# sulaimanvesal/PointCloudUDA

Measured on AMD Instinct MI355X. Metric: adversarial train-step images/sec (seg+3 discr) at 256x256, higher is better.
Workload: dtype bf16x3 MFMA (split-bf16, fp32 accumulate; fp32 storage); 1 GPU; MS-CMRSeg full UDA: UNet(PointNet head) + d1 + d2 + d4, 256x256x1, 4 classes; per_gpu_batch=32, global_batch=32, precision=bf16x3, parallelism=dp1, ranks_in_group=1, collective=none, streams=discriminators concurrent, d_target_forward=replayed from the adversarial pass of the same step, launch=eager (256 host cores for this rank)

## Files before the change

include/pcuda_hip.h:

```cpp
#ifndef PCUDA_HIP_H
#define PCUDA_HIP_H

#include <stddef.h>
#include <stdint.h>

#ifdef __cplusplus
extern "C" {
#endif

#define PCUDA_OK 0
#define PCUDA_E_BADARG (-1)
#define PCUDA_E_UNSUPPORTED (-2)
#define PCUDA_E_LAUNCH (-3)
#define PCUDA_E_WORKSPACE (-4)

#define PCUDA_PREC_BF16X3 0
#define PCUDA_PREC_BF16 1

typedef void* pcuda_stream_t;

#define PCUDA_ABI_VERSION 5
int pcuda_version(void);
size_t pcuda_abi_struct_size(int which);
int pcuda_device_count(void);
const char* pcuda_last_error(void);
const char* pcuda_build_hash(void);
long long pcuda_launch_count(int reset);
long long pcuda_fallback_count(void);
const char* pcuda_last_kernel(void);
int pcuda_clock_probe(unsigned long long* out2_dev, float* sink_dev, int iters, pcuda_stream_t s);

#define PCUDA_FAM_CONV_FWD 0
#define PCUDA_FAM_CONV_WGRAD 1
#define PCUDA_FAM_POINTWISE 2
#define PCUDA_FAM_DENSE_F32 3
#define PCUDA_FAM_COUNT 4
int pcuda_prof_enable(int on);
int pcuda_prof_reset(void);
int pcuda_prof_read(int family, double* ms, double* work, long long* launches);
int pcuda_prof_dump(const char* path);
int pcuda_debug_read_clocks(unsigned long long* out8);

typedef struct pcuda_conv_geom {
  int n;
  int cin, cout;
  int in_h, in_w;
  int out_h, out_w;
  int k, stride, pad, dil;
  int in_up;
} pcuda_conv_geom;

typedef struct pcuda_src {
  const float* p1; long long sn1, sc1; const float* scale1; const float* shift1;
  const float* p2; long long sn2, sc2; const float* scale2; const float* shift2;
  int c1;
} pcuda_src;
typedef struct pcuda_dst {
  float* p1; long long sn1, sc1;
  float* p2; long long sn2, sc2;
  int c1;
} pcuda_dst;

size_t pcuda_conv2d_packed_fwd_bytes(const pcuda_conv_geom* g, int prec);
size_t pcuda_conv2d_packed_dgrad_bytes(const pcuda_conv_geom* g, int prec);
int pcuda_conv2d_pack_fwd(const pcuda_conv_geom* g, int prec, const float* w, void* packed, pcuda_stream_t s);
int pcuda_conv2d_pack_dgrad(const pcuda_conv_geom* g, int prec, const float* w, void* packed, pcuda_stream_t s);
int pcuda_conv2d_pack_all(const pcuda_conv_geom* g, int prec, const float* w, void* packed_fwd, void* packed_dgrad,
                          pcuda_stream_t s);
size_t pcuda_conv2d_pack_job_bytes(void);
int pcuda_conv2d_pack_jobs_fill(const pcuda_conv_geom* g, int prec, const float* w, void* packed_fwd, void* packed_dgrad,
                                void* host_jobs, int max_jobs, int* job_blocks);
int pcuda_conv2d_pack_table(const void* dev_jobs, const int* dev_first_block, int njobs, int total_blocks, pcuda_stream_t s);

int pcuda_conv2d_d1_forward_ok(const pcuda_conv_geom* g);
int pcuda_conv2d_fwd_tiles(const pcuda_conv_geom* g, int prec);
int pcuda_conv2d_forward(const pcuda_conv_geom* g, int prec, const pcuda_src* x, const void* packed_w,
                         const float* bias, float slope, const pcuda_dst* y, float* bn_partials,
                         pcuda_stream_t s);
int pcuda_conv2d_dgrad(const pcuda_conv_geom* g, int prec, const pcuda_src* dy, const void* packed_w_dgrad,
                       const pcuda_dst* dx, int accumulate, pcuda_stream_t s);
int pcuda_conv2d_dgrad_tiles(const pcuda_conv_geom* g, int prec);
int pcuda_conv2d_dgrad_bnred(const pcuda_conv_geom* g, int prec, const pcuda_src* dy, const void* packed_w_dgrad,
                             const pcuda_dst* dx, int accumulate, const float* a, long long a_sn, long long a_sc,
                             const float* mean, const float* invstd, float* red_partials, pcuda_stream_t s);
int pcuda_conv2d_dgrad_lrelu(const pcuda_conv_geom* g, int prec, const pcuda_src* dy, const void* packed_w_dgrad,
                             const pcuda_dst* dx, const float* a, long long a_sn, long long a_sc, float slope,
                             pcuda_stream_t s);
int pcuda_conv2d_dgrad_fold(const pcuda_conv_geom* g, int prec, const pcuda_src* dy, const void* packed_w_dgrad,
                            const pcuda_dst* dx_half, const float* a, long long a_sn, long long a_sc, const float* mean,
                            const float* invstd, float* red_partials, pcuda_stream_t s);
size_t pcuda_conv2d_wgrad_workspace_size(const pcuda_conv_geom* g);
int pcuda_conv2d_wgrad(const pcuda_conv_geom* g, int prec, const pcuda_src* x, const float* dy,
                       long long dy_sn, long long dy_sc, float* dw, float* db, int accumulate,
                       void* workspace, size_t workspace_bytes, pcuda_stream_t s);

#define PCUDA_REDUCE_MAX_JOBS 56
typedef struct {
  const float* partial;
  long long numel;
  float* dw;
  const float* db_partial;
  long long nb;
  float* db;
  int ksplit, nkg, accumulate, ntaps;
} pcuda_reduce_job;
int pcuda_conv2d_wgrad_partial(const pcuda_conv_geom* g, int prec, const pcuda_src* x, const float* dy,
                               long long dy_sn, long long dy_sc, float* dw, float* db, int accumulate,
                               void* workspace, size_t workspace_bytes, pcuda_reduce_job* job, pcuda_stream_t s);
int pcuda_wgrad_reduce_batch(const pcuda_reduce_job* host_jobs, int njobs, pcuda_stream_t s);

int pcuda_bn_finalize(const float* partials, int ntiles, int c, long long count, const float* gamma,
                      const float* beta, float eps, float momentum, float* running_mean, float* running_var,
                      float* mean, float* invstd, float* scale, float* shift, pcuda_stream_t s);
int pcuda_bn_stats(const float* a, long long sn, long long sc, int n, int c, long long hw,
                   float* partials, int* ntiles, pcuda_stream_t s);
#define PCUDA_BN_APPLY_RELU 1
#define PCUDA_BN_APPLY_FMA 2
int pcuda_bn_apply(const float* a, long long a_sn, long long a_sc, const float* scale, const float* shift,
                   int flags, float* y, long long y_sn, long long y_sc, int n, int c, long long hw,
                   pcuda_stream_t s);
int pcuda_bn_bwd_reduce(const float* dy, long long dy_sn, long long dy_sc, const float* dy2, long long dy2_sn,
                        long long dy2_sc, const float* a, long long a_sn, long long a_sc, const float* mean,
                        const float* invstd, const float* scale, const float* shift, int post_relu, int n, int c,
                        long long hw, float* red, int* ntiles, pcuda_stream_t s);
int pcuda_bn_bwd_finalize(const float* red, int ntiles, int c, long long count, const float* gamma,
                          const float* invstd, const float* mean, float* dgamma, float* dbeta, int accumulate,
                          float* coef , pcuda_stream_t s);
int pcuda_bn_bwd_apply(const float* dy, long long dy_sn, long long dy_sc, const float* dy2, long long dy2_sn,
                       long long dy2_sc, const float* a, long long a_sn, long long a_sc, const float* coef,
                       const float* scale, const float* shift, int post_relu, float act_slope, float* dz,
                       long long dz_sn, long long dz_sc, int n, int c, long long hw, pcuda_stream_t s);
int pcuda_lrelu_bwd(const float* dy, long long dy_sn, long long dy_sc, const float* dy2, long long dy2_sn,
                    long long dy2_sc, const float* a, long long a_sn, long long a_sc, float slope, float* dz,
                    long long dz_sn, long long dz_sc, int n, int c, long long hw, pcuda_stream_t s);
int pcuda_channel_sum(const float* dz, long long sn, long long sc, int n, int c, long long hw, float* db,
                      int accumulate, float* workspace, size_t workspace_bytes, pcuda_stream_t s);

int pcuda_maxpool2_fwd(const float* x, long long x_sn, long long x_sc, const float* scale, const float* shift,
                       float* y, long long y_sn, long long y_sc, uint8_t* idx, int n, int c, int h, int w,
                       pcuda_stream_t s);
int pcuda_maxpool2_bwd(const float* dy, long long dy_sn, long long dy_sc, const float* dy2, long long dy2_sn,
                       long long dy2_sc, const uint8_t* idx, float* dx, long long dx_sn, long long dx_sc,
                       int accumulate, int n, int c, int h, int w, pcuda_stream_t s);
typedef struct pcuda_pooled {
  const float* g; long long g_sn, g_sc;
  const float* g2; long long g2_sn, g2_sc;
  const uint8_t* idx;
  int h, w;
} pcuda_pooled;
int pcuda_bn_bwd_reduce_pooled(const pcuda_pooled* pool, const float* dy, long long dy_sn, long long dy_sc, const float* a,
                               long long a_sn, long long a_sc, const float* mean, const float* invstd, int n, int c,
                               float* red, int* ntiles, pcuda_stream_t s);
int pcuda_bn_bwd_apply_pooled(const pcuda_pooled* pool, const float* dy, long long dy_sn, long long dy_sc, const float* a,
                              long long a_sn, long long a_sc, const float* coef, float act_slope, float* dz, long long dz_sn,
                              long long dz_sc, int n, int c, pcuda_stream_t s);
int pcuda_lrelu_bwd_pooled(const pcuda_pooled* pool, const float* dy, long long dy_sn, long long dy_sc, const float* a,
                           long long a_sn, long long a_sc, float slope, float* dz, long long dz_sn, long long dz_sc, int n,
                           int c, pcuda_stream_t s);
int pcuda_upsample2_bwd(const float* dy, long long dy_sn, long long dy_sc, float* dx, long long dx_sn,
                        long long dx_sc, int accumulate, int n, int c, int h, int w, pcuda_stream_t s);
int pcuda_upsample2_bwd_bnred(const float* dy, long long dy_sn, long long dy_sc, float* dx, long long dx_sn,
                              long long dx_sc, int accumulate, const float* a, long long a_sn, long long a_sc,
                              const float* mean, const float* invstd, float* red, int* ntiles, int n, int c, int h, int w,
                              pcuda_stream_t s);
int pcuda_bilinear_fwd(const float* x, long long x_sn, long long x_sc, int n, int c, int h, int w, float* y, int oh,
                       int ow, pcuda_stream_t s);
int pcuda_bilinear_bwd(const float* dy, int n, int c, int oh, int ow, float* dx, long long dx_sn, long long dx_sc,
                       int h, int w, pcuda_stream_t s);
int pcuda_unfold_taps(const float* x, long long x_sn, long long x_sc, int n, int c, int h, int w, int k, int stride,
                      int pad, int dil, float* u, int oh, int ow, pcuda_stream_t s);
int pcuda_add4(const float* a, const float* b, const float* c, const float* d, float* y, long long numel,
               pcuda_stream_t s);
int pcuda_mul(const float* a, const float* b, float* y, long long numel, pcuda_stream_t s);

#define PCUDA_ACT_SIGMOID 0
#define PCUDA_ACT_SOFTMAX 1
int pcuda_entropy_fwd(const float* logits, int mode, float norm, float* ent, float* prob, int n, int c,
                      long long hw, pcuda_stream_t s);
int pcuda_entropy_bwd(const float* logits, int mode, float norm, const float* dent, const float* dprob,
                      float* dlogits, int accumulate, int n, int c, long long hw, pcuda_stream_t s);
int pcuda_entropy_bwd2(const float* logits, int mode, float norm, const float* dent, const float* dprob, const float* dmean,
                       float* dlogits, int accumulate, int n, int c, long long hw, pcuda_stream_t s);
size_t pcuda_sum_all_workspace_size(void);
int pcuda_sum_all(const float* x, long long numel, double scale, float* out, void* workspace, size_t workspace_bytes,
                  pcuda_stream_t s);
size_t pcuda_seg_loss_workspace_size(int n, int c, long long hw);
int pcuda_seg_loss_fwd(const float* logits, const uint8_t* onehot, int mode, int n, int c, long long hw,
                       float* out2, void* workspace, size_t workspace_bytes, pcuda_stream_t s);
int pcuda_seg_loss_bwd(const float* logits, const uint8_t* onehot, int mode, int n, int c, long long hw,
                       const float* g_main, const float* g_jac, float* dlogits, const void* workspace,
                       pcuda_stream_t s);
int pcuda_bce_const_fwd(const float* x, long long numel, float label, float* loss, float* acc, pcuda_stream_t s);
int pcuda_bce_const_bwd(const float* x, long long numel, float label, const float* gout, float gscale, float* dx,
                        pcuda_stream_t s);
size_t pcuda_nn_loss_workspace_floats(int b, int npts);
int pcuda_nn_loss_fwd(const float* x, const float* y, int b, int npts, float* loss, int* idx_ws, float* val_ws,
                      pcuda_stream_t s);
int pcuda_nn_loss_bwd(const float* x, const float* y, int b, int npts, const int* idx_ws, const float* val_ws,
                      const float* gout, float* dx, pcuda_stream_t s);
int pcuda_dice_metric(const float* logits, const uint8_t* onehot, int n, int c, long long hw, float* dice,
                      void* workspace, size_t workspace_bytes, pcuda_stream_t s);
int pcuda_assemble_batch(const float* images_hwc, const int* mask_labels, int b, int h, int w, int c, int crop,
                         int num_classes, float* images_chw, uint8_t* onehot, pcuda_stream_t s);
size_t pcuda_minmax_workspace_size(void);
int pcuda_minmax(const float* x, long long numel, float* out2, void* workspace, size_t workspace_bytes, pcuda_stream_t s);
int pcuda_quantize_u8(const float* x, long long numel, const float* minmax, uint8_t* q, pcuda_stream_t s);
#define PCUDA_AUG_NONE 0
#define PCUDA_AUG_MINMAX 1
#define PCUDA_AUG_DIV255 2
int pcuda_augment_assemble(const void* images_hwc, int images_u8, const int* mask_labels, int b, int h, int w, int c, int crop,
                           int num_classes, const double* inv_mats, const int* order, const int* cval, int rescale,
                           const float* minmax, float* images_chw, uint8_t* onehot, uint8_t* full_mask, int* labels_full,
                           uint8_t* images_u8_full, pcuda_stream_t s);
int pcuda_augment_assemble_dequant(const uint8_t* images_hwc, const int* mask_labels, int b, int h, int w, int c, int crop,
                                   int num_classes, const double* inv_mats, const int* order, const int* cval,
                                   const float* minmax, float* images_chw, uint8_t* onehot, uint8_t* full_mask,
                                   int* labels_full, uint8_t* images_u8_full, pcuda_stream_t s);
#define PCUDA_PHOTO_NOP 0
#define PCUDA_PHOTO_GAUSSIAN_BLUR 1
#define PCUDA_PHOTO_AVERAGE_BLUR 2
#define PCUDA_PHOTO_MEDIAN_BLUR 3
#define PCUDA_PHOTO_CONV3X3 4
#define PCUDA_PHOTO_GAUSSIAN_NOISE 5
#define PCUDA_PHOTO_DROPOUT 6
#define PCUDA_PHOTO_COARSE_DROPOUT 7
#define PCUDA_PHOTO_INVERT 8
#define PCUDA_PHOTO_ADD 9
#define PCUDA_PHOTO_MULTIPLY 10
#define PCUDA_PHOTO_GRAYSCALE 11
size_t pcuda_photometric_workspace_size(int b, int h, int w, int c);
int pcuda_photometric(const uint8_t* in, uint8_t* out, int b, int h, int w, int c, int slots, const int* opcode,
                      const int* iarg, const double* farg, const unsigned long long* seed, void* workspace,
                      size_t workspace_bytes, pcuda_stream_t s);
#define PCUDA_GEO_NOP 0
#define PCUDA_GEO_HOMOGRAPHY 1
#define PCUDA_GEO_ELASTIC 2
#define PCUDA_GEO_PIECEWISE_AFFINE 3
#define PCUDA_GEO_CONSTANT 0
#define PCUDA_GEO_EDGE 1
#define PCUDA_GEO_REFLECT 2
#define PCUDA_GEO_SYMMETRIC 3
#define PCUDA_GEO_WRAP 4
size_t pcuda_geometric_workspace_size(int b, int h, int w, int c, int with_labels);
int pcuda_geometric(const uint8_t* in, uint8_t* out, const int* labels_in, int* labels_out, int b, int h, int w, int c,
                    int slots, const int* opcode, const int* iarg, const double* farg, const unsigned long long* seed,
                    void* workspace, size_t workspace_bytes, pcuda_stream_t s);
int pcuda_geometric_cubic(const uint8_t* in, uint8_t* out, const int* labels_in, int* labels_out, int b, int h, int w, int c,
                          int slots, const int* opcode, const int* iarg, const double* farg, const unsigned long long* seed,
                          void* workspace, size_t workspace_bytes, pcuda_stream_t s);
#define PCUDA_STYLE_NOP 0
#define PCUDA_STYLE_HUE_SATURATION 1
#define PCUDA_STYLE_NOISE_ALPHA_CONV3X3 2
#define PCUDA_STYLE_SUPERPIXELS 3
size_t pcuda_stylize_workspace_size(int b, int h, int w, int c);
int pcuda_stylize(const uint8_t* in, uint8_t* out, int b, int h, int w, int c, int slots, const int* opcode, const int* iarg,
                  const double* farg, const double* table, const unsigned long long* seed, void* workspace,
                  size_t workspace_bytes, pcuda_stream_t s);
size_t pcuda_stylize_connect_workspace_size(int b, int h, int w, int c);
int pcuda_stylize_connect(const uint8_t* in, uint8_t* out, int b, int h, int w, int c, int slots, const int* opcode,
                          const int* iarg, const double* farg, const double* table, const unsigned long long* seed,
                          void* workspace, size_t workspace_bytes, pcuda_stream_t s);
size_t pcuda_stylize_scaled_workspace_size(int b, int h, int w, int c);
int pcuda_stylize_scaled(const uint8_t* in, uint8_t* out, int b, int h, int w, int c, int slots, const int* opcode,
                         const int* iarg, const double* farg, const double* table, const unsigned long long* seed,
                         void* workspace, size_t workspace_bytes, pcuda_stream_t s);
#define PCUDA_PAD_CONSTANT 0
#define PCUDA_PAD_EDGE 1
#define PCUDA_PAD_LINEAR_RAMP 2
#define PCUDA_PAD_MAXIMUM 3
#define PCUDA_PAD_MEAN 4
#define PCUDA_PAD_MEDIAN 5
#define PCUDA_PAD_MINIMUM 6
#define PCUDA_PAD_REFLECT 7
#define PCUDA_PAD_SYMMETRIC 8
#define PCUDA_PAD_WRAP 9
size_t pcuda_crop_pad_workspace_size(int b, int h, int w, int c);
int pcuda_crop_pad(const uint8_t* in, uint8_t* out, const int* labels_in, int* labels_out, int b, int h, int w, int c,
                   const int* opcode, const int* iarg, void* workspace, size_t workspace_bytes, pcuda_stream_t s);
size_t pcuda_match_hist_workspace_size(int b, int h, int w, int c, int is_u8);
int pcuda_match_hist(const void* in, void* out, int is_u8, int b, int h, int w, int c, const double* tvalues,
                     const double* tquantiles, const int* tlen, int tstride, void* workspace, size_t workspace_bytes,
                     pcuda_stream_t s);
size_t pcuda_hist_bank_size(int r, int rh, int rw, int c, int is_u8);
size_t pcuda_hist_bank_workspace_size(int r, int rh, int rw, int c, int is_u8);
int pcuda_hist_bank_build(const void* refs, int is_u8, int r, int rh, int rw, int c, void* bank, size_t bank_bytes, int* flag,
                          void* workspace, size_t workspace_bytes, pcuda_stream_t s);
size_t pcuda_match_hist_bank_workspace_size(int b, int h, int w, int c, int is_u8);
int pcuda_match_hist_bank(const void* in, void* out, int is_u8, int b, int h, int w, int c, const void* bank, int r, int rh,
                          int rw, const int* ref_index, void* workspace, size_t workspace_bytes, pcuda_stream_t s);
size_t pcuda_fourier_bank_size(int r, int c, int radius);
size_t pcuda_fourier_bank_workspace_size(int r, int h, int w, int c, int radius);
int pcuda_fourier_bank_build(const void* refs, int is_u8, int r, int h, int w, int c, int radius, void* bank, size_t bank_bytes,
                             void* workspace, size_t workspace_bytes, pcuda_stream_t s);
size_t pcuda_fourier_adapt_workspace_size(int b, int h, int w, int c, int radius);
int pcuda_fourier_adapt(const void* in, void* out, int is_u8, int b, int h, int w, int c, const void* bank, int r, int radius,
                        const int* ref_index, const int* sample_radius, int clip, double clip_lo, double clip_hi, void* workspace,
                        size_t workspace_bytes, pcuda_stream_t s);
#define PCUDA_CLAHE_U8 0
#define PCUDA_CLAHE_F32X3 1
#define PCUDA_PRE_F32 0
#define PCUDA_PRE_I16 1
#define PCUDA_PRE_U8 2
#define PCUDA_PRE_U8_RAW 3
size_t pcuda_clahe_workspace_size(int n, int tiles_x, int tiles_y);
int pcuda_clahe(const uint8_t* in, void* out, int n, int h, int w, double clip_limit, int tiles_x, int tiles_y, int out_mode,
                void* workspace, size_t workspace_bytes, pcuda_stream_t s);
size_t pcuda_rescale_resize_crop_u8_workspace_size(void);
int pcuda_rescale_resize_crop_u8(const void* in, int in_dtype, int n, int sh, int sw, int resize_h, int resize_w, int crop,
                                 uint8_t* out, void* workspace, size_t workspace_bytes, pcuda_stream_t s);
size_t pcuda_zoom_linear_crop_workspace_size(int zh, int zw, int crop);
int pcuda_zoom_linear_crop(const void* in, int dtype, int n, int sh, int sw, int zh, int zw, int crop, void* out,
// ... 132 lines not shown
```

pointcloududa_amd/_lib.py:

```python
from __future__ import annotations

import ctypes as C
import os

_HERE = os.path.dirname(os.path.abspath(__file__))
LIB_PATH = os.environ.get("PCUDA_LIB") or os.path.join(_HERE, "lib", "libpcuda_hip.so")

PREC_BF16X3, PREC_BF16 = 0, 1
ACT_SIGMOID, ACT_SOFTMAX = 0, 1
OV_DICE_CLASS, OV_DICE_SAMPLE = 1, 2
FAM_CONV_FWD, FAM_CONV_WGRAD, FAM_POINTWISE, FAM_DENSE_F32 = 0, 1, 2, 3

c_f32p = C.c_void_p
i32, i64, f32, f64, vp, sz = C.c_int, C.c_longlong, C.c_float, C.c_double, C.c_void_p, C.c_size_t


class ConvGeom(C.Structure):
    _fields_ = [("n", i32), ("cin", i32), ("cout", i32), ("in_h", i32), ("in_w", i32), ("out_h", i32),
                ("out_w", i32), ("k", i32), ("stride", i32), ("pad", i32), ("dil", i32), ("in_up", i32)]


class ReduceJob(C.Structure):
    _fields_ = [("partial", C.c_void_p), ("numel", C.c_longlong), ("dw", C.c_void_p), ("db_partial", C.c_void_p),
                ("nb", C.c_longlong), ("db", C.c_void_p), ("ksplit", C.c_int), ("nkg", C.c_int), ("accumulate", C.c_int),
                ("ntaps", C.c_int)]


class Src(C.Structure):
    _fields_ = [("p1", vp), ("sn1", i64), ("sc1", i64), ("scale1", vp), ("shift1", vp),
                ("p2", vp), ("sn2", i64), ("sc2", i64), ("scale2", vp), ("shift2", vp), ("c1", i32)]


class Dst(C.Structure):
    _fields_ = [("p1", vp), ("sn1", i64), ("sc1", i64), ("p2", vp), ("sn2", i64), ("sc2", i64), ("c1", i32)]


class Pooled(C.Structure):
    _fields_ = [("g", vp), ("g_sn", i64), ("g_sc", i64), ("g2", vp), ("g2_sn", i64), ("g2_sc", i64), ("idx", vp),
                ("h", i32), ("w", i32)]


_PROTOS = {
    "pcuda_version": (i32, []),
    "pcuda_device_count": (i32, []),
    "pcuda_last_error": (C.c_char_p, []),
    "pcuda_build_hash": (C.c_char_p, []),
    "pcuda_launch_count": (i64, [i32]),
    "pcuda_fallback_count": (i64, []),
    "pcuda_abi_struct_size": (sz, [i32]),
    "pcuda_last_kernel": (C.c_char_p, []),
    "pcuda_clock_probe": (i32, [vp, vp, i32, vp]),
    "pcuda_prof_enable": (i32, [i32]),
    "pcuda_prof_reset": (i32, []),
    "pcuda_prof_read": (i32, [i32, C.POINTER(C.c_double), C.POINTER(C.c_double), C.POINTER(i64)]),
    "pcuda_prof_dump": (i32, [C.c_char_p]),
    "pcuda_debug_read_clocks": (i32, [vp]),
    "pcuda_conv2d_packed_fwd_bytes": (sz, [C.POINTER(ConvGeom), i32]),
    "pcuda_conv2d_packed_dgrad_bytes": (sz, [C.POINTER(ConvGeom), i32]),
    "pcuda_conv2d_pack_fwd": (i32, [C.POINTER(ConvGeom), i32, vp, vp, vp]),
    "pcuda_conv2d_pack_all": (i32, [C.POINTER(ConvGeom), i32, vp, vp, vp, vp]),
    "pcuda_conv2d_pack_dgrad": (i32, [C.POINTER(ConvGeom), i32, vp, vp, vp]),
    "pcuda_conv2d_pack_job_bytes": (sz, []),
    "pcuda_conv2d_pack_jobs_fill": (i32, [C.POINTER(ConvGeom), i32, vp, vp, vp, vp, i32, C.POINTER(i32)]),
    "pcuda_conv2d_pack_table": (i32, [vp, vp, i32, i32, vp]),
    "pcuda_conv2d_fwd_tiles": (i32, [C.POINTER(ConvGeom), i32]),
    "pcuda_conv2d_forward": (i32, [C.POINTER(ConvGeom), i32, C.POINTER(Src), vp, vp, f32, C.POINTER(Dst), vp, vp]),
    "pcuda_conv2d_d1_forward_ok": (i32, [C.POINTER(ConvGeom)]),
    "pcuda_conv2d_dgrad": (i32, [C.POINTER(ConvGeom), i32, C.POINTER(Src), vp, C.POINTER(Dst), i32, vp]),
    "pcuda_conv2d_dgrad_tiles": (i32, [C.POINTER(ConvGeom), i32]),
    "pcuda_conv2d_dgrad_bnred": (i32, [C.POINTER(ConvGeom), i32, C.POINTER(Src), vp, C.POINTER(Dst), i32, vp, i64, i64, vp,
                                       vp, vp, vp]),
    "pcuda_conv2d_dgrad_fold": (i32, [C.POINTER(ConvGeom), i32, C.POINTER(Src), vp, C.POINTER(Dst), vp, i64, i64, vp, vp, vp, vp]),
    "pcuda_conv2d_dgrad_lrelu": (i32, [C.POINTER(ConvGeom), i32, C.POINTER(Src), vp, C.POINTER(Dst), vp, i64, i64, f32, vp]),
    "pcuda_conv2d_wgrad_workspace_size": (sz, [C.POINTER(ConvGeom)]),
    "pcuda_conv2d_wgrad": (i32, [C.POINTER(ConvGeom), i32, C.POINTER(Src), vp, i64, i64, vp, vp, i32, vp, sz, vp]),
    "pcuda_conv2d_wgrad_partial": (i32, [C.POINTER(ConvGeom), i32, C.POINTER(Src), vp, i64, i64, vp, vp, i32, vp, sz,
                                         C.POINTER(ReduceJob), vp]),
    "pcuda_wgrad_reduce_batch": (i32, [C.POINTER(ReduceJob), i32, vp]),
    "pcuda_bn_finalize": (i32, [vp, i32, i32, i64, vp, vp, f32, f32, vp, vp, vp, vp, vp, vp, vp]),
    "pcuda_bn_stats": (i32, [vp, i64, i64, i32, i32, i64, vp, C.POINTER(i32), vp]),
    "pcuda_bn_apply": (i32, [vp, i64, i64, vp, vp, i32, vp, i64, i64, i32, i32, i64, vp]),
    "pcuda_bn_bwd_reduce": (i32, [vp, i64, i64, vp, i64, i64, vp, i64, i64, vp, vp, vp, vp, i32, i32, i32, i64, vp,
                                  C.POINTER(i32), vp]),
    "pcuda_bn_bwd_finalize": (i32, [vp, i32, i32, i64, vp, vp, vp, vp, vp, i32, vp, vp]),
    "pcuda_bn_bwd_apply": (i32, [vp, i64, i64, vp, i64, i64, vp, i64, i64, vp, vp, vp, i32, f32, vp, i64, i64, i32,
                                 i32, i64, vp]),
    "pcuda_lrelu_bwd": (i32, [vp, i64, i64, vp, i64, i64, vp, i64, i64, f32, vp, i64, i64, i32, i32, i64, vp]),
    "pcuda_channel_sum": (i32, [vp, i64, i64, i32, i32, i64, vp, i32, vp, sz, vp]),
    "pcuda_maxpool2_fwd": (i32, [vp, i64, i64, vp, vp, vp, i64, i64, vp, i32, i32, i32, i32, vp]),
    "pcuda_maxpool2_bwd": (i32, [vp, i64, i64, vp, i64, i64, vp, vp, i64, i64, i32, i32, i32, i32, i32, vp]),
    "pcuda_bn_bwd_reduce_pooled": (i32, [C.POINTER(Pooled), vp, i64, i64, vp, i64, i64, vp, vp, i32, i32, vp, C.POINTER(i32), vp]),
    "pcuda_bn_bwd_apply_pooled": (i32, [C.POINTER(Pooled), vp, i64, i64, vp, i64, i64, vp, f32, vp, i64, i64, i32, i32, vp]),
    "pcuda_lrelu_bwd_pooled": (i32, [C.POINTER(Pooled), vp, i64, i64, vp, i64, i64, f32, vp, i64, i64, i32, i32, vp]),
    "pcuda_upsample2_bwd": (i32, [vp, i64, i64, vp, i64, i64, i32, i32, i32, i32, i32, vp]),
    "pcuda_upsample2_bwd_bnred": (i32, [vp, i64, i64, vp, i64, i64, i32, vp, i64, i64, vp, vp, vp, C.POINTER(i32), i32, i32,
                                        i32, i32, vp]),
    "pcuda_bilinear_fwd": (i32, [vp, i64, i64, i32, i32, i32, i32, vp, i32, i32, vp]),
    "pcuda_bilinear_bwd": (i32, [vp, i32, i32, i32, i32, vp, i64, i64, i32, i32, vp]),
    "pcuda_unfold_taps": (i32, [vp, i64, i64, i32, i32, i32, i32, i32, i32, i32, i32, vp, i32, i32, vp]),
    "pcuda_add4": (i32, [vp, vp, vp, vp, vp, i64, vp]),
    "pcuda_mul": (i32, [vp, vp, vp, i64, vp]),
    "pcuda_entropy_fwd": (i32, [vp, i32, f32, vp, vp, i32, i32, i64, vp]),
    "pcuda_entropy_bwd": (i32, [vp, i32, f32, vp, vp, vp, i32, i32, i32, i64, vp]),
    "pcuda_entropy_bwd2": (i32, [vp, i32, f32, vp, vp, vp, vp, i32, i32, i32, i64, vp]),
    "pcuda_sum_all_workspace_size": (sz, []),
    "pcuda_sum_all": (i32, [vp, i64, C.c_double, vp, vp, sz, vp]),
    "pcuda_seg_loss_workspace_size": (sz, [i32, i32, i64]),
    "pcuda_seg_loss_fwd": (i32, [vp, vp, i32, i32, i32, i64, vp, vp, sz, vp]),
    "pcuda_seg_loss_bwd": (i32, [vp, vp, i32, i32, i32, i64, vp, vp, vp, vp, vp]),
    "pcuda_jaccard_workspace_size": (sz, [i32]),
    "pcuda_jaccard_fwd": (i32, [vp, vp, i32, i32, i32, i64, f32, vp, vp, sz, vp]),
    "pcuda_jaccard_bwd": (i32, [vp, i32, i32, i32, i64, f32, vp, vp, vp, vp]),
    "pcuda_seg_loss_ov_workspace_size": (sz, [i32, i32, i64, i32]),
    "pcuda_seg_loss_ov_fwd": (i32, [vp, vp, i32, i32, C.c_double, i32, i32, i64, vp, vp, sz, vp]),
    "pcuda_seg_loss_ov_bwd": (i32, [vp, vp, i32, i32, i32, i32, i64, vp, vp, vp, vp, sz, vp]),
    "pcuda_dice_workspace_size": (sz, [i32, i32, i64, i32]),
    "pcuda_dice_fwd": (i32, [vp, vp, i32, i32, i32, i64, i32, f32, vp, vp, sz, vp]),
    "pcuda_dice_bwd": (i32, [vp, i32, i32, i32, i64, i32, vp, vp, vp, sz, vp]),
    "pcuda_dice_labels_workspace_size": (sz, [i32, i32, i64]),
    "pcuda_dice_labels_fwd": (i32, [vp, vp, i32, i32, i32, i64, f32, vp, vp, vp, sz, vp]),
    "pcuda_dice_labels_bwd": (i32, [vp, vp, i32, i32, i32, i64, vp, vp, vp, sz, vp]),
    "pcuda_bce_const_fwd": (i32, [vp, i64, f32, vp, vp, vp]),
    "pcuda_bce_const_bwd": (i32, [vp, i64, f32, vp, f32, vp, vp]),
    "pcuda_nn_loss_workspace_floats": (sz, [i32, i32]),
    "pcuda_nn_loss_fwd": (i32, [vp, vp, i32, i32, vp, vp, vp, vp]),
    "pcuda_nn_loss_bwd": (i32, [vp, vp, i32, i32, vp, vp, vp, vp, vp]),
    "pcuda_dice_metric": (i32, [vp, vp, i32, i32, i64, vp, vp, sz, vp]),
    "pcuda_assemble_batch": (i32, [vp, vp, i32, i32, i32, i32, i32, i32, vp, vp, vp]),
    "pcuda_minmax_workspace_size": (sz, []),
    "pcuda_minmax": (i32, [vp, i64, vp, vp, sz, vp]),
    "pcuda_augment_assemble": (i32, [vp, i32, vp, i32, i32, i32, i32, i32, i32, vp, vp, vp, i32, vp, vp, vp, vp, vp, vp, vp]),
    "pcuda_quantize_u8": (i32, [vp, i64, vp, vp, vp]),
    "pcuda_augment_assemble_dequant": (i32, [vp, vp, i32, i32, i32, i32, i32, i32, vp, vp, vp, vp, vp, vp, vp, vp, vp, vp]),
    "pcuda_photometric_workspace_size": (sz, [i32, i32, i32, i32]),
    "pcuda_photometric": (i32, [vp, vp, i32, i32, i32, i32, i32, vp, vp, vp, vp, vp, sz, vp]),
    "pcuda_geometric_workspace_size": (sz, [i32, i32, i32, i32, i32]),
    "pcuda_geometric": (i32, [vp, vp, vp, vp, i32, i32, i32, i32, i32, vp, vp, vp, vp, vp, sz, vp]),
    "pcuda_geometric_cubic": (i32, [vp, vp, vp, vp, i32, i32, i32, i32, i32, vp, vp, vp, vp, vp, sz, vp]),
    "pcuda_stylize_workspace_size": (sz, [i32, i32, i32, i32]),
    "pcuda_stylize": (i32, [vp, vp, i32, i32, i32, i32, i32, vp, vp, vp, vp, vp, vp, sz, vp]),
    "pcuda_stylize_connect_workspace_size": (sz, [i32, i32, i32, i32]),
    "pcuda_stylize_connect": (i32, [vp, vp, i32, i32, i32, i32, i32, vp, vp, vp, vp, vp, vp, sz, vp]),
    "pcuda_stylize_scaled_workspace_size": (sz, [i32, i32, i32, i32]),
    "pcuda_stylize_scaled": (i32, [vp, vp, i32, i32, i32, i32, i32, vp, vp, vp, vp, vp, vp, sz, vp]),
    "pcuda_crop_pad_workspace_size": (sz, [i32, i32, i32, i32]),
    "pcuda_crop_pad": (i32, [vp, vp, vp, vp, i32, i32, i32, i32, vp, vp, vp, sz, vp]),
    "pcuda_match_hist_workspace_size": (sz, [i32, i32, i32, i32, i32]),
    "pcuda_match_hist": (i32, [vp, vp, i32, i32, i32, i32, i32, vp, vp, vp, i32, vp, sz, vp]),
    "pcuda_hist_bank_size": (sz, [i32, i32, i32, i32, i32]),
    "pcuda_hist_bank_workspace_size": (sz, [i32, i32, i32, i32, i32]),
    "pcuda_hist_bank_build": (i32, [vp, i32, i32, i32, i32, i32, vp, sz, vp, vp, sz, vp]),
    "pcuda_match_hist_bank_workspace_size": (sz, [i32, i32, i32, i32, i32]),
    "pcuda_match_hist_bank": (i32, [vp, vp, i32, i32, i32, i32, i32, vp, i32, i32, i32, vp, vp, sz, vp]),
    "pcuda_fourier_bank_size": (sz, [i32, i32, i32]),
    "pcuda_fourier_bank_workspace_size": (sz, [i32, i32, i32, i32, i32]),
    "pcuda_fourier_bank_build": (i32, [vp, i32, i32, i32, i32, i32, i32, vp, sz, vp, sz, vp]),
    "pcuda_fourier_adapt_workspace_size": (sz, [i32, i32, i32, i32, i32]),
    "pcuda_fourier_adapt": (i32, [vp, vp, i32, i32, i32, i32, i32, vp, i32, i32, vp, vp, i32, f64, f64, vp, sz, vp]),
    "pcuda_clahe_workspace_size": (sz, [i32, i32, i32]),
    "pcuda_clahe": (i32, [vp, vp, i32, i32, i32, f64, i32, i32, i32, vp, sz, vp]),
    "pcuda_rescale_resize_crop_u8_workspace_size": (sz, []),
    "pcuda_rescale_resize_crop_u8": (i32, [vp, i32, i32, i32, i32, i32, i32, i32, vp, vp, sz, vp]),
    "pcuda_zoom_linear_crop_workspace_size": (sz, [i32, i32, i32]),
    "pcuda_zoom_linear_crop": (i32, [vp, i32, i32, i32, i32, i32, i32, i32, vp, vp, sz, vp]),
    "pcuda_zoom_standardize_workspace_size": (sz, [i32, i32, i32, i32, i32]),
    "pcuda_zoom_standardize": (i32, [vp, i32, i32, i32, i32, i32, i32, i32, i32, vp, vp, vp, sz, vp]),
    "pcuda_zoom_labels_workspace_size": (sz, [i32, i32, i32]),
    "pcuda_zoom_labels": (i32, [vp, i32, i32, i32, i32, i32, i32, i32, i32, vp, i32, vp, vp, sz, vp]),
    "pcuda_volume_slices": (i32, [vp, i32, i64, i64, i64, i64, i32, i32, i32, i32, i32, i32, vp, vp]),
    "pcuda_volume_labels_workspace_size": (sz, []),
    "pcuda_volume_labels": (i32, [vp, i32, i64, i64, i64, i64, i32, i32, i32, i32, i32, i32, vp, i32, i32, vp, vp, vp, sz, vp]),
    "pcuda_volume_restore": (i32, [vp, i32, i32, i32, vp, i32, i64, i64, i64, i64, i32, i32, vp, vp]),
    "pcuda_argmax_labels": (i32, [vp, i32, i64, i64, i32, i32, i64, vp, vp]),
    "pcuda_label_dice": (i32, [vp, vp, i64, i32, vp, vp, sz, vp]),
    "pcuda_area_resize": (i32, [vp, i64, i64, i32, i32, i32, vp, i32, i32, vp]),
    "pcuda_reconstruct_resize_argmax": (i32, [vp, i64, i64, i64, i32, i32, i32, i32, i32, i32, vp, i32, i32, vp]),
    "pcuda_surface_metrics_workspace_size": (sz, [i32, i32, i32, i32, i32, vp]),
    "pcuda_surface_metrics": (i32, [vp, vp, i32, i32, i32, i32, i32, vp, i32, i32, vp, vp, vp, sz, vp]),
    "pcuda_surface_metrics_ext_workspace_size": (sz, [i32, i32, i32, i32, i32, vp]),
    "pcuda_surface_metrics_ext": (i32, [vp, vp, i32, i32, i32, i32, i32, vp, i32, i32, vp, f64, vp, vp, sz, vp]),
    "pcuda_largest_components_workspace_size": (sz, [i32, i32, i32, i32]),
    "pcuda_largest_components": (i32, [vp, i32, i32, i32, i32, i32, i32, vp, vp, sz, vp]),
    "pcuda_linear_fwd": (i32, [vp, vp, vp, vp, i32, i32, i32, vp]),
    "pcuda_linear_bwd_x": (i32, [vp, vp, vp, i32, i32, i32, i32, vp]),
    "pcuda_linear_bwd_w_workspace_size": (sz, [i32, i32, i32]),
    "pcuda_linear_bwd_w": (i32, [vp, vp, vp, vp, i32, i32, i32, i32, vp, sz, vp]),
    "pcuda_conv1d_k1_fwd_tiles": (i32, [i32, i32]),
    "pcuda_conv1d_k1_fwd": (i32, [vp, vp, vp, vp, i32, i32, i32, i32, vp, vp]),
    "pcuda_conv1d_k1_dgrad": (i32, [vp, vp, vp, i32, i32, i32, i32, vp]),
    "pcuda_conv1d_k1_wgrad_workspace_size": (sz, [i32, i32, i32, i32]),
    "pcuda_conv1d_k1_wgrad": (i32, [vp, vp, vp, vp, i32, i32, i32, i32, i32, vp, sz, vp]),
    "pcuda_max_points_fwd": (i32, [vp, i32, i32, i32, vp, vp, vp]),
    "pcuda_max_points_bwd": (i32, [vp, vp, i32, i32, i32, vp, vp]),
    "pcuda_bn1d_fwd": (i32, [vp, i64, i32, i32, vp, vp, f32, f32, vp, vp, vp, vp, vp, vp, i32, vp, i64, vp]),
    "pcuda_bn1d_bwd": (i32, [vp, i64, vp, i64, i32, i32, vp, vp, vp, vp, vp, i32, f32, vp, vp, i32, vp, i64, vp]),
    "pcuda_bn_bwd_reduce_maxpts": (i32, [vp, vp, vp, vp, vp, vp, vp, i32, i32, i32, i32, vp, vp]),
    "pcuda_bn_bwd_apply_maxpts": (i32, [vp, vp, vp, vp, vp, vp, i32, f32, vp, i32, i32, i32, vp]),
    "pcuda_bmm": (i32, [vp, vp, vp, i32, i32, i32, i32, i32, i32, i32, vp]),
    "pcuda_surface_vertices": (i32, [vp, i32, i32, i32, vp, i32, vp, vp, sz, vp]),
    "pcuda_surface_vertices_mc": (i32, [vp, i32, i32, i32, vp, i32, vp, vp]),
    "pcuda_fps": (i32, [vp, vp, vp, i32, i32, i32, vp, vp]),
    "pcuda_adam_step": (i32, [vp, vp, vp, vp, i64, f32, f32, f32, f32, f32, i32, f32, vp]),
    "pcuda_adam_step_dev": (i32, [vp, vp, vp, vp, i64, f32, f32, f32, f32, f32, vp, f32, vp]),
    "pcuda_sgd_step": (i32, [vp, vp, vp, i64, f32, f32, f32, i32, f32, vp]),
    "pcuda_grad_norm": (i32, [vp, C.POINTER(i64), i32, f32, f32, i32, vp, vp, vp, sz, vp]),
    "pcuda_adam_step_guarded": (i32, [vp, vp, vp, vp, i64, f32, f32, f32, f32, f32, vp, f32, vp, i32, vp]),
    "pcuda_sgd_step_guarded": (i32, [vp, vp, vp, i64, f32, f32, f32, vp, i32, f32, vp, i32, vp]),
}

EXPORTED_SYMBOLS = tuple(_PROTOS.keys())
_lib = None


PCUDA_E_UNSUPPORTED = -2
PCUDA_ABI_VERSION = 5
GUARD_MAX_RANGES, GUARD_RECORD_WORDS, GRAD_NORM_WORKSPACE_BYTES = 16, 8, 16384


def lib():
    global _lib
    if _lib is None:
        if not os.path.exists(LIB_PATH):
            raise RuntimeError("libpcuda_hip.so is missing at %s: build it with pointcloududa_amd/csrc/Makefile "
                               "(there is no CPU fallback)" % LIB_PATH)
        handle = C.CDLL(LIB_PATH)
        for name, (res, args) in _PROTOS.items():
            fn = getattr(handle, name)
            fn.restype, fn.argtypes = res, args
        ver = handle.pcuda_version()
        if ver != PCUDA_ABI_VERSION:
            raise RuntimeError("libpcuda_hip.so at %s has ABI version %d, this binding is written against %d: rebuild it "
                               "(python -c 'import __graft_entry__ as g; g.build()')" % (LIB_PATH, ver, PCUDA_ABI_VERSION))
        for which, st in enumerate((ConvGeom, Src, Dst, Pooled, ReduceJob)):
            if handle.pcuda_abi_struct_size(which) != C.sizeof(st):
                raise RuntimeError("libpcuda_hip.so: sizeof(%s) is %d in the library, %d in the binding: header / library mismatch"
                                   % (st.__name__, handle.pcuda_abi_struct_size(which), C.sizeof(st)))
        _lib = handle
    return _lib


def source_hash(csrc: str) -> str:
    import glob
    import hashlib
    h = hashlib.sha256()
    files = sorted(glob.glob(os.path.join(csrc, "*.hip")) + glob.glob(os.path.join(csrc, "*.h")) +
                   [os.path.join(csrc, "Makefile"), os.path.join(os.path.dirname(os.path.dirname(csrc)), "include", "pcuda_hip.h")])
# ... 24 lines not shown
```

pointcloududa_amd/csrc/conv_host.h:

```cpp
#pragma once
#include <stdlib.h>
#include <string.h>
#include "conv_igemm.h"

static const int LDS_HARD = 160 * 1024;

static inline bool geom_ok(const pcuda_conv_geom* g) {
  if (!g || g->n <= 0 || g->cin <= 0 || g->cout <= 0 || g->k <= 0 || g->stride <= 0 || g->dil <= 0 || g->pad < 0)
    return false;
  if (g->k * g->k > IG_MAX_TAPS) return false;
  const int oh = (g->in_h + 2 * g->pad - g->dil * (g->k - 1) - 1) / g->stride + 1;
  const int ow = (g->in_w + 2 * g->pad - g->dil * (g->k - 1) - 1) / g->stride + 1;
  if (oh != g->out_h || ow != g->out_w || oh <= 0 || ow <= 0) return false;
  if (g->in_up && ((g->in_h & 1) || (g->in_w & 1))) return false;
  return true;
}

static inline bool src_ok(const pcuda_src* s, int c) {
  if (!s || !s->p1 || s->c1 <= 0 || s->c1 > c) return false;
  if (s->c1 < c && !s->p2) return false;
  return true;
}
static inline bool dst_ok(const pcuda_dst* d, int c) {
  if (!d || !d->p1 || d->c1 <= 0 || d->c1 > c) return false;
  if (d->c1 < c && !d->p2) return false;
  return true;
}

struct TapSet {
  int n;
  signed char dy[IG_MAX_TAPS], dx[IG_MAX_TAPS], src[IG_MAX_TAPS];
  int dy_min, dy_max, dx_min, dx_max;
  void finish() {
    dy_min = dx_min = 127; dy_max = dx_max = -127;
    for (int i = 0; i < n; ++i) {
      if (dy[i] < dy_min) dy_min = dy[i];
      if (dy[i] > dy_max) dy_max = dy[i];
      if (dx[i] < dx_min) dx_min = dx[i];
      if (dx[i] > dx_max) dx_max = dx[i];
    }
    if (n == 0) dy_min = dy_max = dx_min = dx_max = 0;
  }
};

static inline TapSet fwd_taps(const pcuda_conv_geom* g) {
  TapSet t = {};
  for (int ky = 0; ky < g->k; ++ky)
    for (int kx = 0; kx < g->k; ++kx) {
      t.dy[t.n] = (signed char)(ky * g->dil - g->pad);
      t.dx[t.n] = (signed char)(kx * g->dil - g->pad);
      t.src[t.n] = (signed char)(ky * g->k + kx);
      ++t.n;
    }
  t.finish();
  return t;
}

static inline int posmod(int a, int m) { return ((a % m) + m) % m; }

static inline TapSet dgrad_taps(const pcuda_conv_geom* g, int ry, int rx) {
  TapSet t = {};
  const int s = g->stride;
  for (int ky = 0; ky < g->k; ++ky) {
    const int vy = ry + g->pad - ky * g->dil;
    if (posmod(vy, s) != 0) continue;
    for (int kx = 0; kx < g->k; ++kx) {
      const int vx = rx + g->pad - kx * g->dil;
      if (posmod(vx, s) != 0) continue;
      t.dy[t.n] = (signed char)(vy / s);
      t.dx[t.n] = (signed char)(vx / s);
      t.src[t.n] = (signed char)(ky * g->k + kx);
      ++t.n;
    }
  }
  t.finish();
  return t;
}

static inline bool dgrad_pair_enabled() {
  static int on = -1;
  if (on < 0) { const char* e = getenv("PCUDA_DGRAD_PAIR"); on = (e && !atoi(e)) ? 0 : 1; }
  return on != 0;
}
static inline bool dgrad_pair_ok(const pcuda_conv_geom* g) {
  if (g->stride != 2 || g->in_up || g->cin <= 5 || !dgrad_pair_enabled()) return false;
  for (int ry = 0; ry < 2; ++ry) {
    const TapSet a = dgrad_taps(g, ry, 0), b = dgrad_taps(g, ry, 1);
    if (a.n < 1 || a.n != b.n || 2 * a.n > IG_MAX_TAPS) return false;
    for (int i = 0; i < a.n; ++i)
      if (a.dy[i] != b.dy[i] || a.dx[i] != b.dx[i]) return false;
  }
  return true;
}
static inline TapSet dgrad_pair_taps(const pcuda_conv_geom* g, int ry) {
  TapSet t = dgrad_taps(g, ry, 0);
  const TapSet b = dgrad_taps(g, ry, 1);
  for (int i = 0; i < b.n; ++i) t.src[t.n + i] = b.src[i];
  return t;
}

static inline int tile_width_candidates(int lw, int tile_px, int* out) {
  int n = 0;
  for (int t = 8; t <= 256 && t <= tile_px; t <<= 1) out[n++] = t;
  for (int parts = 1; parts <= 4; ++parts) {
    const int t = (lw + parts - 1) / parts;
    if (t >= 4 && t <= 256 && t <= tile_px) {
      bool dup = false;
      for (int i = 0; i < n; ++i) dup |= out[i] == t;
      if (!dup) out[n++] = t;
    }
  }
  return n;
}


static inline bool fast_src_ok(const pcuda_src* x, int cin) {
  const long long lim = 1ll << 30;
  const int c1 = x->c1 < cin ? x->c1 : cin;
  if (c1 < cin && (c1 & 31)) return false;
  if ((long long)(c1 + 32) * x->sc1 * 4 >= lim) return false;
  if (c1 < cin && (long long)(cin - c1 + 32) * x->sc2 * 4 >= lim) return false;
  return true;
}

static inline bool aligned16(const void* p, long long sn, long long sc) { return (((uintptr_t)p) & 15) == 0 && (sn & 3) == 0 && (sc & 3) == 0; }

static inline bool fast_dst_ok(const pcuda_dst* y, int cout) {
  const long long lim = 1ll << 30;
  const int c1 = y->c1 < cout ? y->c1 : cout;
  if (c1 < cout && (c1 & 7)) return false;
  if ((long long)(c1 + 64) * y->sc1 * 4 >= lim) return false;
  if (c1 < cout && (long long)(cout - c1 + 64) * y->sc2 * 4 >= lim) return false;
  return true;
}

struct IgemmPlan {
  int npb, tw, th, tiles_x, tiles_y, ih_t, iw_t, clamp, x_cap, tg;
  size_t lds;
  int fat;
  int w8;
  int te;
};

static inline bool te_dst_ok(const pcuda_dst* y, int cout, int out_w, int lw, int tw, int ox_mul, int ox_off) {
  if (ox_mul != 1 || ox_off != 0 || (tw & 3) || (out_w & 3) || (lw & 3)) return false;
  if (((uintptr_t)y->p1 & 15) || (y->sc1 & 3) || (y->sn1 & 3)) return false;
  if (y->c1 < cout && (((uintptr_t)y->p2 & 15) || (y->sc2 & 3) || (y->sn2 & 3))) return false;
  return true;
}


struct IgemmParams;
struct PackParams;
bool ap_layer_ok(const pcuda_conv_geom* g, int rows, int red, int prec);
size_t ap_layer_packed_bytes(int rows, int red);
bool ap_fill_pack(PackParams& p, const float* w, unsigned char* out, int rows, int red, long long s_row, long long s_red,
                  const TapSet& taps);
int ap_launch_pack(const float* w, unsigned char* out, int rows, int red, long long s_row, long long s_red, const TapSet& taps,
                   hipStream_t s);
bool ap_map_ok(int n, int h, int w, int rows);
int ap_tiles(int n, int h, int w);
int ap_try_launch(const IgemmParams& p, const TapSet& taps, const unsigned char* image, hipStream_t s, int* rc);

bool rs_layer_ok(const pcuda_conv_geom* g, int rows, int red, int prec);
bool rs_map_ok(int n, int h, int w);
int rs_tiles(int n, int h, int w);
int rs_try_launch(const IgemmParams& p, int prec, const TapSet& taps, hipStream_t s, int* rc);

static inline size_t packed_elems(int rows, int red, int ntaps, int prec) {
  const int co_tile = 32 * ig_co_blks(rows);
  const int n_co_tiles = cdiv(rows, co_tile), nchunks = cdiv(red, 32);
  return (size_t)n_co_tiles * nchunks * ntaps * co_tile * (ig_rec_bytes(prec == PCUDA_PREC_BF16X3) / 2);
}

enum { SIDE_FWD = 0, SIDE_DGRAD = 1 };
enum { IMG_ORDINARY = 0, IMG_PAIR = 1, IMG_AP = 2 };
struct PackedImage {
  int kind;
  int rows, red;
  long long s_row, s_red;
  int ry, rx;
  size_t off, bytes;
  TapSet taps;
};
struct PackedLayout {
  int n;
  size_t bytes;
  PackedImage img[IG_MAX_TAPS + 1];
  const PackedImage* ap() const { return n > 0 && img[n - 1].kind == IMG_AP ? &img[n - 1] : nullptr; }
  const PackedImage* cls(int ry, int rx) const {
    for (int i = 0; i < n; ++i)
      if (img[i].kind != IMG_AP && img[i].ry == ry && img[i].rx == rx) return &img[i];
    return nullptr;
  }
};
static inline void packed_layout(const pcuda_conv_geom* g, int prec, int side, PackedLayout* L) {
  const int kk = g->k * g->k;
  const bool fwd = side == SIDE_FWD;
  const int rows = fwd ? g->cout : g->cin, red = fwd ? g->cin : g->cout;
  const long long s_row = fwd ? (long long)g->cin * kk : kk, s_red = fwd ? kk : (long long)g->cin * kk;
  L->n = 0; L->bytes = 0;
  auto add = [&](int kind, int r, const TapSet& t, int ry, int rx) {
    PackedImage& im = L->img[L->n++];
    im.kind = kind; im.rows = r; im.red = red; im.s_row = s_row; im.s_red = s_red; im.ry = ry; im.rx = rx; im.taps = t;
    im.off = L->bytes;
    im.bytes = kind == IMG_AP ? ap_layer_packed_bytes(r, red) : packed_elems(r, red, t.n, prec) * 2;
    L->bytes += im.bytes;
  };
  if (fwd) {
    add(IMG_ORDINARY, rows, fwd_taps(g), 0, 0);
  } else if (dgrad_pair_ok(g)) {
    for (int ry = 0; ry < 2; ++ry) add(IMG_PAIR, 2 * rows, dgrad_pair_taps(g, ry), ry, 0);
    return;
  } else {
    for (int ry = 0; ry < g->stride; ++ry)
      for (int rx = 0; rx < g->stride; ++rx) {
        const TapSet t = dgrad_taps(g, ry, rx);
        if (t.n) add(IMG_ORDINARY, rows, t, ry, rx);
      }
  }
  if (ap_layer_ok(g, rows, red, prec)) add(IMG_AP, rows, L->img[0].taps, 0, 0);
}

int direct_fwd_tiles(const pcuda_conv_geom* g);
int direct_forward(const pcuda_conv_geom* g, int prec, const pcuda_src* x, const void* packed_w, long long w_lo_off,
                   const float* bias, float slope, const pcuda_dst* y, float* bn_partials, hipStream_t s, int* rc);
int direct_dgrad_tiles(const pcuda_conv_geom* g);
int direct_dgrad(const pcuda_conv_geom* g, int prec, const pcuda_src* dy, const void* packed_w_dgrad, const pcuda_dst* dx,
                 int accumulate, hipStream_t s, int* rc, const float* red_a = nullptr, long long red_sn = 0,
                 long long red_sc = 0, const float* red_mean = nullptr, const float* red_invstd = nullptr,
                 float* red = nullptr);
int direct_d1_dgrad(const pcuda_conv_geom* g, int prec, const pcuda_src* dy, const void* packed_w_dgrad, const pcuda_dst* dx,
                    int accumulate, size_t cls_elems, hipStream_t s, int* rc);
int direct_d1_forward(const pcuda_conv_geom* g, int prec, const pcuda_src* x, const void* packed_w, const float* bias,
                      float slope, const pcuda_dst* y, float* bn_partials, hipStream_t s, int* rc);
int direct_d5_forward(const pcuda_conv_geom* g, int prec, const pcuda_src* x, const void* packed_w, const float* bias,
                      float slope, const pcuda_dst* y, float* bn_partials, hipStream_t s, int* rc);

struct WgradCall {
  const pcuda_conv_geom* g;
  int prec;
  const pcuda_src* x;
  const float* dy;
  long long dy_sn, dy_sc;
  float* dw;
  float* db;
  int accumulate;
  void* workspace;
  hipStream_t s;
  pcuda_reduce_job* defer;
};
enum { WGRAD_NOT_TAKEN = 1 };

struct WgradSlabs {
  float* partial;
  float* db_partial;
  long long welems;
  int slices, ntaps;
};
static inline size_t wgrad_slab_bytes(const pcuda_conv_geom* g, int slices) {
  return ((size_t)slices * g->cout * g->cin * g->k * g->k + (size_t)slices * g->cout) * sizeof(float) + 256;
}
WgradSlabs wgrad_slabs(const WgradCall& c, int slices, int ntaps);
int wgrad_finish(const WgradCall& c, const WgradSlabs& sl);
int launch_wgrad_reduce(const float* partial, long long numel, int ksplit, float* dw, int accumulate, int ntaps,
                        const float* db_partial, long long nb, float* db, hipStream_t s);

int direct_wgrad_slices(const pcuda_conv_geom* g);
int direct_wgrad(const WgradCall& c);
size_t direct_d1_wgrad_bytes(const pcuda_conv_geom* g);
int direct_d1_wgrad(const WgradCall& c);
int wgrad3r_slices(const pcuda_conv_geom* g);
int wgrad3r_wgrad(const WgradCall& c);
int wgrad3_slices(const pcuda_conv_geom* g);
int wgrad3_wgrad(const WgradCall& c);
int wgrad1_slices(const pcuda_conv_geom* g);
int wgrad1_wgrad(const WgradCall& c);
```

pointcloududa_amd/csrc/conv_igemm.hip:

```cpp
#include <algorithm>
#include <stdlib.h>

#include "conv_igemm.h"
#include "conv_host.h"

#define PACK_MAX_JOBS 5
struct PackJobs {
  int n;
  PackParams p[PACK_MAX_JOBS];
};
__global__ void pack_multi_kernel(const PackJobs jobs) {
  const PackParams& p = jobs.p[blockIdx.y];
  const long long total = (long long)p.n_co_tiles * p.nchunks * p.ntaps * p.co_tile * p.rec;
  for (long long idx = blockIdx.x * (long long)blockDim.x + threadIdx.x; idx < total;
       idx += (long long)gridDim.x * blockDim.x) {
    int col = (int)(idx % p.rec);
    long long rest = idx / p.rec;
    int row = (int)(rest % p.co_tile); rest /= p.co_tile;
    int t = (int)(rest % p.ntaps); rest /= p.ntaps;
    int ch = (int)(rest % p.nchunks);
    int cot = (int)(rest / p.nchunks);
    const bool is_lo = p.rec > IG_REC && col >= 32;
    const int cc = is_lo ? col - 32 : col;
    int r = cot * p.co_tile + row, c = ch * 32 + cc;
// ... 135 lines not shown
  p.pair = im.kind == IMG_PAIR ? 1 : 0;
  memcpy(p.tap_src, im.taps.src, sizeof(p.tap_src));
  p.co_tile = 32 * ig_co_blks(im.rows);
  p.n_co_tiles = cdiv(im.rows, p.co_tile);
  p.nchunks = cdiv(im.red, 32);
  p.rec = ig_rec_bytes(prec == PCUDA_PREC_BF16X3) / 2;
  return true;
}

int launch_pack_jobs(const PackJobs& jobs, size_t max_elems, int max_blocks, hipStream_t s) {
  const int blocks = (int)std::min<size_t>((max_elems + 255) / 256, max_blocks);
  hipLaunchKernelGGL(pack_multi_kernel, dim3(blocks, jobs.n), dim3(256), 0, s, jobs);
  PCUDA_CHECK_LAUNCH("pack_multi_kernel");
  return PCUDA_OK;
}

int launch_pack(const float* w, void* buf, int prec, const PackedImage& im, hipStream_t s) {
  if (im.kind == IMG_AP)
    return ap_launch_pack(w, (unsigned char*)buf + im.off, im.rows, im.red, im.s_row, im.s_red, im.taps, s);
  PackJobs jobs = {};
  jobs.n = 1;
  fill_pack(jobs.p[0], w, buf, prec, im);
  return launch_pack_jobs(jobs, im.bytes / 2, 4096, s);
}

int pack_side(const pcuda_conv_geom* g, int prec, int side, const float* w, void* packed, hipStream_t s) {
  PackedLayout L;
  packed_layout(g, prec, side, &L);
  int rc = PCUDA_OK;
  for (int i = 0; i < L.n && rc == PCUDA_OK; ++i) rc = launch_pack(w, packed, prec, L.img[i], s);
  return rc;
}

int plan_lds(bool x3, int co_tile, int x_cap, int ntaps, int mode, int* tg_out, size_t* lds_out) {
  const bool fat = mode != 0;
  const size_t rec = ig_rec_bytes(x3), vecs = rec / 16;
  const size_t xb = (size_t)x_cap * rec;
  const size_t wtap = (size_t)co_tile * rec;
  const size_t epi = 4 * (size_t)co_tile * 2 * sizeof(float);
  const size_t tab = 1024;
  if (ntaps < 1) ntaps = 1;
  const int slots = mode == 2 ? (x3 ? 11 : 6) * 512 : (x3 ? (co_tile == 32 ? 8 : 7) : (co_tile == 32 ? 4 : 3)) * 256;
  const int cap = slots / (int)(co_tile * vecs);
  const size_t budgets[3] = {54528, 81920, 163840};
  for (int b = fat ? 2 : 0; b < 3; ++b) {
    if (xb + tab >= budgets[b]) continue;
    int fit = (int)((budgets[b] - xb - tab) / wtap);
    if (fit > cap) fit = cap;
    const int need = b == 0 ? (ntaps < 3 ? ntaps : 3) : 1;
    if (fit < need) continue;
    const int tg = fit > ntaps ? ntaps : fit;
    size_t total = xb + (size_t)tg * wtap + tab;
    if (total < epi) total = epi;
    *tg_out = tg; *lds_out = total;
    return 0;
  }
  return -1;
}


int plan_igemm_mode(int rows, int lh, int lw, int in_h, int in_w, int in_step, const TapSet& taps, bool x3,
                    int mode_env, IgemmPlan* best, int n = 0) {
  const int co_tile = 32 * ig_co_blks(rows);
  long long best_key = -1;
  for (int npb = 2; npb >= 1; --npb) {
    const int TP = 128 * npb;
    int cand[16];
    const int nc = tile_width_candidates(lw, TP, cand);
    for (int ci = 0; ci < nc; ++ci) {
      IgemmPlan pl;
      pl.npb = npb; pl.tw = cand[ci]; pl.th = TP / pl.tw;
      if (pl.th < 1) continue;
      pl.tiles_x = cdiv(lw, pl.tw);
      pl.tiles_y = cdiv(lh, pl.th);
      pl.ih_t = (pl.th - 1) * in_step + (taps.dy_max - taps.dy_min) + 1;
      pl.iw_t = (pl.tw - 1) * in_step + (taps.dx_max - taps.dx_min) + 1;
      const int full = pl.ih_t * pl.iw_t;
      const int clipped = (pl.ih_t < in_h ? pl.ih_t : in_h) * (pl.iw_t < in_w ? pl.iw_t : in_w) + 1;
      bool ok = false;
      for (int attempt = 0; attempt < 2 && !ok; ++attempt) {
        pl.clamp = attempt == 0 ? ((clipped * 2 <= full) ? 1 : 0) : 1;
        pl.x_cap = pl.clamp ? clipped : full;
        int mode = mode_env;
        if (mode == 2) {
          const int ihc = (pl.clamp && pl.ih_t > in_h) ? in_h : pl.ih_t;
          const bool fits = pl.x_cap <= 1024 && ihc * ((pl.iw_t + 6) / 4) <= 256;
          if (!fits || (npb == 1 && co_tile == 32)) mode = 0;
        }
        pl.fat = mode == 1 ? 1 : 0;
        pl.w8 = mode == 2 ? 1 : 0;
        ok = plan_lds(x3, co_tile, pl.x_cap, taps.n, mode, &pl.tg, &pl.lds) == 0;
        if (pl.clamp) break;
      }
      if (!ok) continue;
      const long long slots = (long long)pl.tiles_x * pl.tiles_y * TP;
      const long long halo = (long long)pl.x_cap * 64 / TP;
      const long long groups = (taps.n + pl.tg - 1) / pl.tg;
      const long long items = (long long)n * pl.tiles_x * pl.tiles_y * cdiv(rows, co_tile);
      static int nofill = -1;
      if (nofill < 0) { const char* e = getenv("PCUDA_NO_UNDERFILL"); nofill = (e && atoi(e)) ? 1 : 0; }
      const long long underfill = (!nofill && n > 0 && items < 256) ? (256 - items + 63) / 64 : 0;
      const long long key = (slots << 28) + (underfill << 25) + ((groups > 3 ? groups : 3) << 22) + ((pl.tw & 31) ? (1ll << 20) : 0) +
                            (halo << 8) + (npb == 1 ? 1 : 0);
      if (best_key < 0 || key < best_key) { best_key = key; *best = pl; }
    }
  }
  return best_key < 0 ? -1 : 0;
}

int plan_igemm(int rows, int red, int n, int lh, int lw, int in_h, int in_w, int in_step, const TapSet& taps, bool x3,
               IgemmPlan* best, bool allow8 = true) {
  const int mode_env = allow8 ? ig_plan_mode() : 0;
  const bool single_chunk = red <= 32;
  IgemmPlan p0;
  const int rc0 = plan_igemm_mode(rows, lh, lw, in_h, in_w, in_step, taps, x3, mode_env == 2 ? 0 : mode_env, &p0);
  if (mode_env != 2) { *best = p0; return rc0; }
  IgemmPlan p8;
  const int rc8 = plan_igemm_mode(rows, lh, lw, in_h, in_w, in_step, taps, x3, 2, &p8, n);
  if (rc8 < 0 || !p8.w8) { *best = p0; return rc0; }
  if (rc0 < 0) { *best = p8; return rc8; }
  const long long t0 = (long long)p0.tiles_x * p0.tiles_y, t8 = (long long)p8.tiles_x * p8.tiles_y;
  const long long items = (long long)n * (t0 < t8 ? t0 : t8) * cdiv(rows, 32 * ig_co_blks(rows));
  const bool wstay = rows <= 64 && taps.n <= p8.tg && single_chunk;
  const bool use8 = p0.lds > 81920 || items <= 320 || (wstay && ig_wstay_mode());
  *best = use8 ? p8 : p0;
  return 0;
}

enum { ROUTE_DIRECT, ROUTE_AP, ROUTE_RS, ROUTE_IGEMM };
struct ConvRoute {
  int family, tiles;
};
ConvRoute conv_route(const pcuda_conv_geom* g, int prec, int side, bool plan = true) {
  const bool fwd = side == SIDE_FWD;
  if (!fwd && g->stride != 1) return {ROUTE_IGEMM, 0};
  const int rows = fwd ? g->cout : g->cin, red = fwd ? g->cin : g->cout;
  if (const int d = fwd ? direct_fwd_tiles(g) : direct_dgrad_tiles(g)) return {ROUTE_DIRECT, d};
  if (ap_layer_ok(g, rows, red, prec) && ap_map_ok(g->n, g->in_h, g->in_w, rows)) return {ROUTE_AP, ap_tiles(g->n, g->in_h, g->in_w)};
  if (rs_layer_ok(g, rows, red, prec) && rs_map_ok(g->n, g->in_h, g->in_w)) return {ROUTE_RS, rs_tiles(g->n, g->in_h, g->in_w)};
  if (!plan) return {ROUTE_IGEMM, -1};
  IgemmPlan pl;
  const bool x3 = prec == PCUDA_PREC_BF16X3;
  const int rc = fwd ? plan_igemm(rows, red, g->n, g->out_h, g->out_w, g->in_h, g->in_w, g->stride, fwd_taps(g), x3, &pl)
                     : plan_igemm(rows, red, g->n, g->in_h, g->in_w, g->out_h, g->out_w, 1, dgrad_taps(g, 0, 0), x3, &pl);
  return {ROUTE_IGEMM, rc < 0 ? 0 : g->n * pl.tiles_x * pl.tiles_y};
}

int launch_igemm(IgemmParams& p, int prec, const TapSet& taps, hipStream_t s, const unsigned char* ap_image = nullptr,
                 const ConvRoute* expect = nullptr) {
  {
    int rc;
    if (ap_image && prec == PCUDA_PREC_BF16X3 && ap_try_launch(p, taps, ap_image, s, &rc)) return rc;
    if (p.cin == 32 && p.cout == 32 && rs_try_launch(p, prec, taps, s, &rc)) return rc;
  }
  const bool x3 = prec == PCUDA_PREC_BF16X3;
  const int co_blks = ig_co_blks(p.cout);
  const int co_tile = 32 * co_blks;
  IgemmPlan pl;
  if (plan_igemm(p.cout, p.cin, p.n, p.lh, p.lw, p.in_h, p.in_w, p.in_step, taps, x3, &pl, true) < 0)
    PCUDA_FAIL(PCUDA_E_UNSUPPORTED, "igemm: no tile of this convolution fits LDS (in_step %d, tap span %d)",
               p.in_step, taps.dy_max - taps.dy_min);
  if (p.stats && expect && expect->tiles >= 0 && (long long)pl.tiles_x * pl.tiles_y * p.n != expect->tiles)
    PCUDA_FAIL(PCUDA_E_UNSUPPORTED, "conv: tensors the %s kernel cannot address on a map whose ordinary plan has other tiles",
               expect->family == ROUTE_AP ? "anti-phase" : "row-streaming");
  p.n_co_tiles = cdiv(p.cout, co_tile);
  p.nchunks = cdiv(p.cin, 32);
  p.tw = pl.tw; p.th = pl.th; p.tmagic = 65536 / pl.tw + 1; p.tiles_x = pl.tiles_x; p.tiles_y = pl.tiles_y;
  auto fmagic = [](int d) -> unsigned { return d <= 1 ? 0u : (unsigned)((1ull << 32) / (unsigned)d) + 1u; };
  p.m_cot = fmagic(p.n_co_tiles); p.m_tx = fmagic(pl.tiles_x); p.m_ty = fmagic(pl.tiles_y);
  p.ntaps = taps.n;
  memcpy(p.dy, taps.dy, sizeof(p.dy));
  memcpy(p.dx, taps.dx, sizeof(p.dx));
  p.dy_min = taps.dy_min; p.dx_min = taps.dx_min;
  p.ih_t = pl.ih_t; p.iw_t = pl.iw_t; p.clamp = pl.clamp; p.tg = pl.tg;
  {
    static int dbg = -1;
    if (dbg < 0) { const char* e = getenv("PCUDA_DBG"); dbg = e ? atoi(e) : 0; }
    p.dbg = dbg;
    static unsigned long long* clkbuf = nullptr;
    if ((dbg & 128) && !clkbuf && hipMalloc((void**)&clkbuf, 64) == hipSuccess) (void)hipMemset(clkbuf, 0, 64);
    p.dbg_clk = clkbuf;
    g_dbg_clk_host = clkbuf;
  }
  const double flops = 2.0 * p.n * (double)p.lh * p.lw * p.cout * (double)p.cin * taps.n;
  char tag[160];
  snprintf(tag, sizeof(tag), "igemm n%d red%d rows%d %dx%d taps%d step%d up%d tw%d npb%d clamp%d tg%d w8%d lds%zu", p.n,
           p.cin, p.cout, p.lh, p.lw, taps.n, p.in_step, p.in_shift, pl.tw, pl.npb, pl.clamp, pl.tg, pl.w8, pl.lds);
  ProfScope prof(PCUDA_FAM_CONV_FWD, flops, s, tag);
  static int nopipe = -1;
  if (nopipe < 0) { const char* e = getenv("PCUDA_NOPIPE"); nopipe = e ? atoi(e) : 0; }
  const int max_pix = pl.clamp ? pl.x_cap - 1 : pl.ih_t * pl.iw_t;
  int pf = (max_pix + 255) / 256;
  {
    static int noxq = -1;
    if (noxq < 0) { const char* e = getenv("PCUDA_NOXQ"); noxq = e ? atoi(e) : 0; }
    const int ih = (pl.clamp && pl.ih_t > p.in_h) ? p.in_h : pl.ih_t;
    const int pfq = (ih * ((pl.iw_t + 6) / 4) + 63) / 64;
    p.xq = (!noxq && (p.in_w & 3) == 0 && p.in_shift == 0 && pfq <= 3) ? 1 : 0;
    if (p.xq) pf = pfq;
    if (pl.w8) pf = p.xq ? (ih * ((pl.iw_t + 6) / 4) + 127) / 128 : (max_pix + 511) / 512;
  }
  const long long total_items = (long long)p.n_co_tiles * p.n * pl.tiles_x * pl.tiles_y;
  const int max_div = std::max(p.n_co_tiles, std::max(pl.tiles_x, pl.tiles_y));
  const bool pipe = !nopipe && p.ntaps > 0 && fast_src_ok(&p.x, p.cin) && fast_dst_ok(&p.y, p.cout) &&
                    (pf <= 2 || (pf == 3 && !pl.w8 && (pl.npb == 1 || pl.fat))) && total_items < (1ll << 32) / max_div;
  {
    static int note = -1;
    if (note < 0) { const char* e = getenv("PCUDA_NOTE"); note = e ? atoi(e) : 0; }
    const bool fold_ok = p.fold && p.ox_mul == 1 && p.ox_off == 0 && !(pl.tw & 3) && !(p.lw & 3) && !(p.out_w & 1) &&
                         !((uintptr_t)p.y.p1 & 7) && !(p.y.sc1 & 1) && !(p.y.sn1 & 1) &&
                         (p.y.c1 >= p.cout || (!((uintptr_t)p.y.p2 & 7) && !(p.y.sc2 & 1) && !(p.y.sn2 & 1)));
    pl.te = (pipe && !pl.w8 && !note &&
             (p.fold ? fold_ok : te_dst_ok(&p.y, p.cout, p.out_w, p.lw, pl.tw, p.ox_mul, p.ox_off))) ? 1 : 0;
    if (pl.te) {
      const size_t rec = ig_rec_bytes(x3), wtap = (size_t)co_tile * rec;
      const size_t need = (size_t)16384 * pl.npb + (size_t)co_tile * 32;
      const size_t have = (size_t)pl.x_cap * rec + (size_t)pl.tg * wtap;
      if (have < need) {
        const int add = (int)((need - have + rec - 1) / rec);
        pl.x_cap += add;
        pl.lds += (size_t)add * rec;
      }
    }
  }
  if (p.fold && !(pipe && pl.te && !pl.w8 && pl.npb == 2 && pl.tw == 32 && pl.th == 8 && !pl.clamp && !p.accumulate && !p.pair))
    PCUDA_FAIL(PCUDA_E_UNSUPPORTED, "conv2d_dgrad_fold: this geometry does not run on the 32 x 8-tile transposed-epilogue kernel");
  if (p.mask_a && (pl.te || p.accumulate || p.stats || p.bias || p.fold || p.y.c1 < (p.cout >> p.pair)))
    PCUDA_FAIL(PCUDA_E_UNSUPPORTED, "conv2d_dgrad_lrelu: this geometry does not run on a plain-epilogue kernel");
  if (p.red_a && !(pipe && pl.te))
    PCUDA_FAIL(PCUDA_E_UNSUPPORTED, "conv2d_dgrad_bnred: this geometry does not run on the transposed-epilogue kernel");
  return x3 ? igemm_dispatch_x3(p, pl, co_blks, pf, pipe, s) : igemm_dispatch_bf16(p, pl, co_blks, pf, pipe, s);
}

}

static size_t packed_bytes(const pcuda_conv_geom* g, int prec, int side) {
  if (!geom_ok(g)) return 0;
  PackedLayout L;
  packed_layout(g, prec, side, &L);
  return L.bytes;
}
extern "C" size_t pcuda_conv2d_packed_fwd_bytes(const pcuda_conv_geom* g, int prec) { return packed_bytes(g, prec, SIDE_FWD); }
extern "C" size_t pcuda_conv2d_packed_dgrad_bytes(const pcuda_conv_geom* g, int prec) { return packed_bytes(g, prec, SIDE_DGRAD); }

extern "C" int pcuda_conv2d_pack_fwd(const pcuda_conv_geom* g, int prec, const float* w, void* packed,
                                     pcuda_stream_t s) {
  if (!geom_ok(g) || !w || !packed) PCUDA_FAIL(PCUDA_E_BADARG, "pack_fwd: bad geometry or null pointer");
  return pack_side(g, prec, SIDE_FWD, w, packed, (hipStream_t)s);
}

extern "C" int pcuda_conv2d_pack_dgrad(const pcuda_conv_geom* g, int prec, const float* w, void* packed,
                                       pcuda_stream_t s) {
  if (!geom_ok(g) || !w || !packed) PCUDA_FAIL(PCUDA_E_BADARG, "pack_dgrad: bad geometry or null pointer");
  return pack_side(g, prec, SIDE_DGRAD, w, packed, (hipStream_t)s);
}

extern "C" int pcuda_conv2d_pack_all(const pcuda_conv_geom* g, int prec, const float* w, void* packed_fwd,
                                     void* packed_dgrad, pcuda_stream_t s) {
  if (!geom_ok(g) || !w || !packed_fwd) PCUDA_FAIL(PCUDA_E_BADARG, "pack_all: bad geometry or null pointer");
  if (g->stride * g->stride + 1 > PACK_MAX_JOBS) {
    int rc = pcuda_conv2d_pack_fwd(g, prec, w, packed_fwd, s);
    if (rc == PCUDA_OK && packed_dgrad) rc = pcuda_conv2d_pack_dgrad(g, prec, w, packed_dgrad, s);
    return rc;
  }
  void* const buf[2] = {packed_fwd, packed_dgrad};
  PackedLayout L[2];
  PackJobs jobs = {};
  size_t max_elems = 0;
  for (int side = 0; side < 2 && buf[side]; ++side) {
    packed_layout(g, prec, side, &L[side]);
    for (int i = 0; i < L[side].n; ++i) {
      const PackedImage& im = L[side].img[i];
      if (im.kind == IMG_AP) continue;
      fill_pack(jobs.p[jobs.n++], w, buf[side], prec, im);
      max_elems = std::max(max_elems, im.bytes / 2);
    }
  }
  int rc = launch_pack_jobs(jobs, max_elems, 2048, (hipStream_t)s);
  for (int side = 0; side < 2 && buf[side] && rc == PCUDA_OK; ++side)
    if (const PackedImage* im = L[side].ap()) rc = launch_pack(w, buf[side], prec, *im, (hipStream_t)s);
  return rc;
}

extern "C" int pcuda_conv2d_fwd_tiles(const pcuda_conv_geom* g, int prec) {
  return geom_ok(g) ? conv_route(g, prec, SIDE_FWD).tiles : 0;
}

static IgemmParams dgrad_params(const pcuda_conv_geom* g, const pcuda_src* dy, const pcuda_dst* dx, const void* packed,
                                const PackedImage* im, int lh, int lw, int mul, int oy_off, int ox_off, int accumulate) {
  IgemmParams p;
  memset(&p, 0, sizeof(p));
  p.x = *dy; p.cin = g->cout;
  p.in_h = g->out_h; p.in_w = g->out_w; p.in_shift = 0; p.in_row = g->out_w;
  p.y = *dx; p.cout = im ? im->rows : g->cin; p.out_w = g->in_w;
  p.lh = lh; p.lw = lw;
  p.oy_mul = p.ox_mul = mul; p.oy_off = oy_off; p.ox_off = ox_off;
  p.in_step = 1;
  p.wpack = (const uint16_t*)((const unsigned char*)packed + (im ? im->off : 0)); p.w_lo_off = 0;
  p.bias = nullptr; p.slope = 1.f; p.accumulate = accumulate; p.stats = nullptr;
  p.n = g->n;
  return p;
}
static const unsigned char* image_ptr(const void* packed, const PackedImage* im) {
  return im ? (const unsigned char*)packed + im->off : nullptr;
}

extern "C" int pcuda_conv2d_forward(const pcuda_conv_geom* g, int prec, const pcuda_src* x, const void* packed_w,
                                    const float* bias, float slope, const pcuda_dst* y, float* bn_partials,
                                    pcuda_stream_t s) {
  if (!geom_ok(g)) PCUDA_FAIL(PCUDA_E_BADARG, "conv2d_forward: inconsistent geometry");
  if (!src_ok(x, g->cin) || !dst_ok(y, g->cout) || !packed_w) PCUDA_FAIL(PCUDA_E_BADARG, "conv2d_forward: bad tensors");
  if (prec != PCUDA_PREC_BF16X3 && prec != PCUDA_PREC_BF16) PCUDA_FAIL(PCUDA_E_BADARG, "conv2d_forward: bad precision");
  {
    int rc;
    if (direct_forward(g, prec, x, packed_w, 0, bias, slope, y,
                       bn_partials, (hipStream_t)s, &rc))
      return rc;
    if (direct_d5_forward(g, prec, x, packed_w, bias, slope, y, bn_partials, (hipStream_t)s, &rc)) return rc;
    if (direct_d1_forward(g, prec, x, packed_w, bias, slope, y, bn_partials, (hipStream_t)s, &rc)) return rc;
  }
  PackedLayout L;
  packed_layout(g, prec, SIDE_FWD, &L);
  IgemmParams p;
  memset(&p, 0, sizeof(p));
  p.x = *x; p.cin = g->cin;
  p.in_h = g->in_h; p.in_w = g->in_w; p.in_shift = g->in_up ? 1 : 0; p.in_row = g->in_w >> p.in_shift;
  p.y = *y; p.cout = g->cout; p.out_w = g->out_w;
  p.lh = g->out_h; p.lw = g->out_w;
  p.oy_mul = p.ox_mul = 1; p.oy_off = p.ox_off = 0;
  p.in_step = g->stride;
  p.wpack = (const uint16_t*)image_ptr(packed_w, &L.img[0]);
  p.w_lo_off = 0;
  p.bias = bias; p.slope = slope; p.accumulate = 0; p.stats = bn_partials;
  p.n = g->n;
  const ConvRoute route = bn_partials ? conv_route(g, prec, SIDE_FWD, false) : ConvRoute{ROUTE_IGEMM, -1};
  return launch_igemm(p, prec, L.img[0].taps, (hipStream_t)s, image_ptr(packed_w, L.ap()), &route);
}

static int dgrad_impl(const pcuda_conv_geom* g, int prec, const pcuda_src* dy, const void* packed_w_dgrad,
                      const pcuda_dst* dx, int accumulate, const float* mask_a, long long mask_sn, float mask_slope,
                      pcuda_stream_t s) {
  if (!geom_ok(g)) PCUDA_FAIL(PCUDA_E_BADARG, "conv2d_dgrad: inconsistent geometry");
  if (!src_ok(dy, g->cout) || !dst_ok(dx, g->cin) || !packed_w_dgrad) PCUDA_FAIL(PCUDA_E_BADARG, "conv2d_dgrad: bad tensors");
  if (prec != PCUDA_PREC_BF16X3 && prec != PCUDA_PREC_BF16) PCUDA_FAIL(PCUDA_E_BADARG, "conv2d_dgrad: bad precision");
  PackedLayout L;
  packed_layout(g, prec, SIDE_DGRAD, &L);
  if (!mask_a) {
    int rc;
    if (direct_dgrad(g, prec, dy, packed_w_dgrad, dx, accumulate, (hipStream_t)s, &rc)) return rc;
    if (direct_d1_dgrad(g, prec, dy, packed_w_dgrad, dx, accumulate, L.img[0].bytes / 2, (hipStream_t)s, &rc)) return rc;
  }
  const int st = g->stride;
  const bool pair = L.img[0].kind == IMG_PAIR;
  const TapSet none = {};
  for (int ry = 0; ry < st; ++ry)
    for (int rx = 0; rx < (pair ? 1 : st); ++rx) {
      const PackedImage* im = L.cls(ry, rx);
      const int lh = (g->in_h - ry + st - 1) / st, lw = (g->in_w - rx + st - 1) / st;
      if (lh <= 0 || lw <= 0) continue;
      IgemmParams p = dgrad_params(g, dy, dx, packed_w_dgrad, im, lh, lw, st, ry, rx, accumulate);
      if (pair) { p.pair = 1; p.lw2 = g->in_w / 2; }
      p.mask_a = mask_a; p.mask_sn = mask_sn; p.mask_slope = mask_slope;
      int rc = launch_igemm(p, prec, im ? im->taps : none, (hipStream_t)s, mask_a ? nullptr : image_ptr(packed_w_dgrad, L.ap()));
      if (rc) return rc;
    }
  return PCUDA_OK;
}

extern "C" int pcuda_conv2d_dgrad(const pcuda_conv_geom* g, int prec, const pcuda_src* dy, const void* packed_w_dgrad,
                                  const pcuda_dst* dx, int accumulate, pcuda_stream_t s) {
  return dgrad_impl(g, prec, dy, packed_w_dgrad, dx, accumulate, nullptr, 0, 1.f, s);
}

extern "C" int pcuda_conv2d_dgrad_lrelu(const pcuda_conv_geom* g, int prec, const pcuda_src* dy, const void* packed_w_dgrad,
                                        const pcuda_dst* dx, const float* a, long long a_sn, long long a_sc, float slope,
                                        pcuda_stream_t s) {
  if (!a || !dx) PCUDA_FAIL(PCUDA_E_BADARG, "conv2d_dgrad_lrelu: bad tensors");
  if (dx->c1 < g->cin || a_sc != dx->sc1 || g->in_up)
    PCUDA_FAIL(PCUDA_E_UNSUPPORTED, "conv2d_dgrad_lrelu: one NCHW destination with the activation's plane stride");
  if (conv_route(g, prec, SIDE_DGRAD, false).family == ROUTE_AP)
    PCUDA_FAIL(PCUDA_E_UNSUPPORTED, "conv2d_dgrad_lrelu: this layer's data gradient runs on the anti-phase kernel");
  return dgrad_impl(g, prec, dy, packed_w_dgrad, dx, 0, a, a_sn, slope, s);
}

extern "C" int pcuda_debug_read_clocks(unsigned long long* out8) {
  unsigned long long z[8] = {0, 0, 0, 0, 0, 0, 0, 0};
  if (!g_dbg_clk_host) { memcpy(out8, z, sizeof(z)); return 0; }
  if (hipMemcpy(out8, g_dbg_clk_host, sizeof(z), hipMemcpyDeviceToHost) != hipSuccess) return -1;
  if (hipMemcpy(g_dbg_clk_host, z, sizeof(z), hipMemcpyHostToDevice) != hipSuccess) return -1;
  return 0;
}

extern "C" int pcuda_conv2d_dgrad_tiles(const pcuda_conv_geom* g, int prec) {
  return geom_ok(g) ? conv_route(g, prec, SIDE_DGRAD).tiles : 0;
}

static int launch_dgrad_stats(IgemmParams& p, const pcuda_conv_geom* g, int prec, const void* packed, const PackedLayout& L,
                              hipStream_t s) {
  const ConvRoute route = conv_route(g, prec, SIDE_DGRAD, false);
  return launch_igemm(p, prec, L.img[0].taps, s, image_ptr(packed, L.ap()), &route);
}

extern "C" int pcuda_conv2d_dgrad_bnred(const pcuda_conv_geom* g, int prec, const pcuda_src* dy, const void* packed_w_dgrad,
                                        const pcuda_dst* dx, int accumulate, const float* a, long long a_sn, long long a_sc,
                                        const float* mean, const float* invstd, float* red_partials, pcuda_stream_t s) {
  if (!geom_ok(g)) PCUDA_FAIL(PCUDA_E_BADARG, "conv2d_dgrad_bnred: inconsistent geometry");
  if (!src_ok(dy, g->cout) || !dst_ok(dx, g->cin) || !packed_w_dgrad || !a || !mean || !invstd || !red_partials)
    PCUDA_FAIL(PCUDA_E_BADARG, "conv2d_dgrad_bnred: bad tensors");
  if (prec != PCUDA_PREC_BF16X3 && prec != PCUDA_PREC_BF16) PCUDA_FAIL(PCUDA_E_BADARG, "conv2d_dgrad_bnred: bad precision");
  if (g->stride != 1 || g->in_up || (((uintptr_t)a) & 15) || (a_sn & 3) || (a_sc & 3))
    PCUDA_FAIL(PCUDA_E_UNSUPPORTED, "conv2d_dgrad_bnred: stride-1 layers with 16-byte aligned activations only");
  if (direct_dgrad_tiles(g)) {
    int rc;
    if (direct_dgrad(g, prec, dy, packed_w_dgrad, dx, accumulate, (hipStream_t)s, &rc, a, a_sn, a_sc, mean, invstd, red_partials))
      return rc;
    PCUDA_FAIL(PCUDA_E_UNSUPPORTED, "conv2d_dgrad_bnred: 1x1 layer with tensors the direct kernel does not take");
  }
  PackedLayout L;
  packed_layout(g, prec, SIDE_DGRAD, &L);
  IgemmParams p = dgrad_params(g, dy, dx, packed_w_dgrad, &L.img[0], g->in_h, g->in_w, 1, 0, 0, accumulate);
  p.stats = red_partials;
  p.red_a = a; p.red_sn = a_sn; p.red_sc = a_sc; p.red_mean = mean; p.red_invstd = invstd;
  return launch_dgrad_stats(p, g, prec, packed_w_dgrad, L, (hipStream_t)s);
}

extern "C" int pcuda_conv2d_dgrad_fold(const pcuda_conv_geom* g, int prec, const pcuda_src* dy, const void* packed_w_dgrad,
                                       const pcuda_dst* dx_half, const float* a, long long a_sn, long long a_sc,
                                       const float* mean, const float* invstd, float* red_partials, pcuda_stream_t s) {
  if (!geom_ok(g)) PCUDA_FAIL(PCUDA_E_BADARG, "conv2d_dgrad_fold: inconsistent geometry");
  if (!src_ok(dy, g->cout) || !dst_ok(dx_half, g->cin) || !packed_w_dgrad) PCUDA_FAIL(PCUDA_E_BADARG, "conv2d_dgrad_fold: bad tensors");
  if (prec != PCUDA_PREC_BF16X3 && prec != PCUDA_PREC_BF16) PCUDA_FAIL(PCUDA_E_BADARG, "conv2d_dgrad_fold: bad precision");
  if (a && (!mean || !invstd || !red_partials)) PCUDA_FAIL(PCUDA_E_BADARG, "conv2d_dgrad_fold: reduce operands missing");
  if (!g->in_up || g->stride != 1 || (g->in_h & 1) || (g->in_w & 3) || direct_dgrad_tiles(g) ||
      (a && ((((uintptr_t)a) & 7) || (a_sn & 1) || (a_sc & 1))))
    PCUDA_FAIL(PCUDA_E_UNSUPPORTED, "conv2d_dgrad_fold: stride-1 MFMA layers behind a nearest-x2 fold, rows of 4k logical pixels");
  PackedLayout L;
  packed_layout(g, prec, SIDE_DGRAD, &L);
  IgemmParams p = dgrad_params(g, dy, dx_half, packed_w_dgrad, &L.img[0], g->in_h, g->in_w, 1, 0, 0, 0);
  p.fold = 1; p.out_w = g->in_w >> 1;
  if (a) {
    p.stats = red_partials;
    p.red_a = a; p.red_sn = a_sn; p.red_sc = a_sc; p.red_mean = mean; p.red_invstd = invstd;
  }
  return launch_dgrad_stats(p, g, prec, packed_w_dgrad, L, (hipStream_t)s);
}

extern "C" size_t pcuda_conv2d_pack_job_bytes(void) { return sizeof(PackParams); }

extern "C" int pcuda_conv2d_pack_jobs_fill(const pcuda_conv_geom* g, int prec, const float* w, void* packed_fwd,
                                           void* packed_dgrad, void* host_jobs, int max_jobs, int* job_blocks) {
  if (!geom_ok(g) || !w || !packed_fwd || !host_jobs || max_jobs < 1 || !job_blocks)
    PCUDA_FAIL(PCUDA_E_BADARG, "pack_jobs_fill: bad arguments");
  if (prec != PCUDA_PREC_BF16X3 && prec != PCUDA_PREC_BF16) PCUDA_FAIL(PCUDA_E_BADARG, "pack_jobs_fill: bad precision");
  PackParams* jobs = (PackParams*)host_jobs;
  void* const buf[2] = {packed_fwd, packed_dgrad};
  int nj = 0;
  for (int side = 0; side < 2 && buf[side]; ++side) {
    PackedLayout L;
    packed_layout(g, prec, side, &L);
    for (int i = 0; i < L.n; ++i, ++nj) {
      if (nj >= max_jobs) PCUDA_FAIL(PCUDA_E_BADARG, "pack_jobs_fill: more layouts than job slots");
      if (!fill_pack(jobs[nj], w, buf[side], prec, L.img[i]))
        PCUDA_FAIL(PCUDA_E_BADARG, "pack_jobs_fill: anti-phase image of a layer that is not 3x3");
      job_blocks[nj] = pack_table_blocks(jobs[nj]);
    }
  }
  return nj;
}

extern "C" int pcuda_conv2d_pack_table(const void* dev_jobs, const int* dev_first_block, int njobs, int total_blocks,
                                       pcuda_stream_t s) {
  if (!dev_jobs || !dev_first_block || njobs < 1 || total_blocks < 1) PCUDA_FAIL(PCUDA_E_BADARG, "pack_table: bad arguments");
  hipLaunchKernelGGL(pack_table_kernel, dim3(total_blocks), dim3(256), 0, (hipStream_t)s, (const PackParams*)dev_jobs,
                     dev_first_block, njobs);
  PCUDA_CHECK_LAUNCH("pack_table_kernel");
  return PCUDA_OK;
}
```

pointcloududa_amd/kernels.py:

```python
from __future__ import annotations

import ctypes as C
import os
import threading
import weakref
from typing import Optional, Tuple

import torch

from . import _lib as L
from ._lib import ACT_SIGMOID, ACT_SOFTMAX, PREC_BF16, PREC_BF16X3, ConvGeom, Dst, Src, check

_PREC = {"bf16x3": PREC_BF16X3, "bf16": PREC_BF16}
_precision = _PREC.get(os.environ.get("PCUDA_PRECISION", "bf16x3").lower(), PREC_BF16X3)


def set_precision(name: str) -> None:
    global _precision
    _precision = _PREC[name.lower()]


def get_precision() -> str:
    return "bf16x3" if _precision == PREC_BF16X3 else "bf16"

# ... 48 lines not shown
def _out(what, out, like, name="out"):
    if out is None:
        return torch.empty_like(like)
    if not torch.is_tensor(out) or not out.is_cuda or out.dtype != like.dtype or out.shape != like.shape or \
            not out.is_contiguous():
        raise ValueError("%s: %s must be a contiguous %s tensor of shape %s"
                         % (what, name, str(like.dtype).replace("torch.", ""), list(like.shape)))
    return out


def _labels_io(what, labels, labels_out, shape):
    if labels is None:
        return None, None
    _req(labels, torch.int32)
    labels = labels.contiguous()
    if tuple(labels.shape) != shape:
        raise ValueError("%s: label shape %r does not match the images" % (what, tuple(labels.shape)))
    return labels, _out(what, labels_out, labels, "labels_out")


def _planes(t: torch.Tensor) -> Tuple[int, int, int, int, int]:
    _req(t)
    n, c = t.shape[0], t.shape[1]
    hw = 1
    for d in t.shape[2:]:
        hw *= d
    exp = 1
    for d in range(t.dim() - 1, 1, -1):
        if t.shape[d] != 1 and t.stride(d) != exp:
            raise ValueError("tensor planes must be dense (shape %s strides %s)" % (tuple(t.shape), t.stride()))
        exp *= t.shape[d]
    return n, c, hw, t.stride(0), t.stride(1)


class TA:
    __slots__ = ("t", "scale", "shift")

    def __init__(self, t, scale=None, shift=None):
        self.t, self.scale, self.shift = t, scale, shift


def _as_ta(x):
    return x if isinstance(x, TA) else TA(x)


def make_src(a, b=None) -> Src:
    a = _as_ta(a)
    _, c1, _, sn1, sc1 = _planes(a.t)
    s = Src()
    s.p1, s.sn1, s.sc1, s.scale1, s.shift1, s.c1 = a.t.data_ptr(), sn1, sc1, _ptr(a.scale), _ptr(a.shift), c1
    if b is not None:
        b = _as_ta(b)
        _, _, _, sn2, sc2 = _planes(b.t)
        s.p2, s.sn2, s.sc2, s.scale2, s.shift2 = b.t.data_ptr(), sn2, sc2, _ptr(b.scale), _ptr(b.shift)
    return s


def make_dst(a: torch.Tensor, b: Optional[torch.Tensor] = None) -> Dst:
    _, c1, _, sn1, sc1 = _planes(a)
    d = Dst()
    d.p1, d.sn1, d.sc1, d.c1 = a.data_ptr(), sn1, sc1, c1
    if b is not None:
        _, _, _, sn2, sc2 = _planes(b)
        d.p2, d.sn2, d.sc2 = b.data_ptr(), sn2, sc2
    return d


_fuse_bnred = os.environ.get("PCUDA_BNRED", "1") != "0"
_fold_dgrad = os.environ.get("PCUDA_FOLD_DGRAD", "1") != "0"


def upsample_red_only(dx, bnred):
    return dx, None


_conv_ops = weakref.WeakSet()


class ConvOp:

    def __init__(self, cin, cout, k, stride=1, pad=0, dil=1, in_up=False):
        self.cin, self.cout, self.k, self.stride, self.pad, self.dil, self.in_up = cin, cout, k, stride, pad, dil, in_up
        self._pk = {}
        self._last_fwd = None
        _conv_ops.add(self)
        self.pack_dgrad_with_fwd = os.environ.get("PCUDA_PACK_ALL", "1") != "0"
        self.owner = None

    def out_hw(self, in_h, in_w):
        f = lambda v: (v + 2 * self.pad - self.dil * (self.k - 1) - 1) // self.stride + 1
        return f(in_h), f(in_w)

    def geom(self, n, in_h, in_w) -> ConvGeom:
        oh, ow = self.out_hw(in_h, in_w)
        return ConvGeom(n, self.cin, self.cout, in_h, in_w, oh, ow, self.k, self.stride, self.pad, self.dil,
                        1 if self.in_up else 0)

    def _packed(self, kind: str, w: torch.Tensor, g: ConvGeom):
        key = (kind, _precision)
        hit = self._pk.get(key)
        gen = getattr(self.owner, "_wgen", 0)
        if hit is not None and hit[0] == w.data_ptr() and hit[1] == w._version and hit[2] == gen:
            return hit[3]
        _req(w)
        if not w.is_contiguous():
            raise ValueError("conv weight must be contiguous OIHW")
        lib = L.lib()
        if kind == "fwd":
            nbytes = lib.pcuda_conv2d_packed_fwd_bytes(C.byref(g), _precision)
        else:
            nbytes = lib.pcuda_conv2d_packed_dgrad_bytes(C.byref(g), _precision)
        if nbytes == 0:
            raise RuntimeError("conv geometry rejected by libpcuda_hip")
        buf = hit[3] if (hit is not None and hit[3].numel() == nbytes) else torch.empty(nbytes, dtype=torch.uint8, device=w.device)
        if kind == "fwd" and self.pack_dgrad_with_fwd:
            dkey = ("dgrad", _precision)
            dhit = self._pk.get(dkey)
            dbytes = lib.pcuda_conv2d_packed_dgrad_bytes(C.byref(g), _precision)
            dbuf = dhit[3] if (dhit is not None and dhit[3].numel() == dbytes) else torch.empty(
                dbytes, dtype=torch.uint8, device=w.device)
            check(lib.pcuda_conv2d_pack_all(C.byref(g), _precision, w.data_ptr(), buf.data_ptr(), dbuf.data_ptr(),
                                            _stream()), "pack_all")
            self._pk[dkey] = (w.data_ptr(), w._version, gen, dbuf)
        else:
            fn = lib.pcuda_conv2d_pack_fwd if kind == "fwd" else lib.pcuda_conv2d_pack_dgrad
            check(fn(C.byref(g), _precision, w.data_ptr(), buf.data_ptr(), _stream()), "pack_" + kind)
        self._pk[key] = (w.data_ptr(), w._version, gen, buf)
        if kind == "fwd":
            self._last_fwd = (w, g)
        return buf

    def forward(self, x, w, b, slope, in_h, in_w, x2=None, out=None, want_stats=False):
        xa = _as_ta(x)
        n = xa.t.shape[0]
        g = self.geom(n, in_h, in_w)
        if out is None:
            out = torch.empty((n, self.cout, g.out_h, g.out_w), dtype=torch.float32, device=w.device)
        pk = self._packed("fwd", w, g)
        lib = L.lib()
        partials, nt = None, 0
        if want_stats:
            nt = lib.pcuda_conv2d_fwd_tiles(C.byref(g), _precision)
            partials = torch.empty((nt, self.cout, 2), dtype=torch.float32, device=w.device)
        src, dst = make_src(xa, x2), make_dst(out)
        rc = lib.pcuda_conv2d_forward(C.byref(g), _precision, C.byref(src), pk.data_ptr(), _ptr(b), float(slope),
                                      C.byref(dst), _ptr(partials), _stream())
        if rc == L.PCUDA_E_UNSUPPORTED and want_stats:
            check(lib.pcuda_conv2d_forward(C.byref(g), _precision, C.byref(src), pk.data_ptr(), _ptr(b), float(slope),
                                           C.byref(dst), None, _stream()), "conv2d_forward")
            partials, nt, _ = bn_stats(out)
            return out, partials, nt
        check(rc, "conv2d_forward")
        return out, partials, nt

    def dgrad(self, dy, w, in_h, in_w, dx=None, dx2=None, accumulate=False, bnred=None):
        n = dy.shape[0]
        g = self.geom(n, in_h, in_w)
        if dx is None:
            dx = torch.empty((n, self.cin, in_h, in_w), dtype=torch.float32, device=dy.device)
        pk = self._packed("dgrad", w, g)
        src, dst = make_src(dy), make_dst(dx, dx2)
        if bnred is not None:
            a, st = bnred
            lib = L.lib()
            nt = lib.pcuda_conv2d_dgrad_tiles(C.byref(g), _precision) if (_fuse_bnred and dx2 is None) else 0
            if nt > 0:
                _, _, _, asn, asc = _planes(a)
                red = torch.empty((nt, self.cin, 2), dtype=torch.float32, device=dy.device)
                rc = lib.pcuda_conv2d_dgrad_bnred(C.byref(g), _precision, C.byref(src), pk.data_ptr(), C.byref(dst),
                                                  1 if accumulate else 0, a.data_ptr(), asn, asc, st.mean.data_ptr(),
                                                  st.invstd.data_ptr(), red.data_ptr(), _stream())
                if rc == 0:
                    return dx, (red, nt)
                if rc != L.PCUDA_E_UNSUPPORTED:
                    check(rc, "conv2d_dgrad_bnred")
            check(lib.pcuda_conv2d_dgrad(C.byref(g), _precision, C.byref(src), pk.data_ptr(), C.byref(dst),
                                         1 if accumulate else 0, _stream()), "conv2d_dgrad")
            return dx, None
        check(L.lib().pcuda_conv2d_dgrad(C.byref(g), _precision, C.byref(src), pk.data_ptr(), C.byref(dst),
                                         1 if accumulate else 0, _stream()), "conv2d_dgrad")
        return dx

    def dgrad_lrelu(self, dy, w, in_h, in_w, a, slope):
        if _fuse_lrelu_dgrad and self.k > 1 and a.is_contiguous():
            n = dy.shape[0]
            g = self.geom(n, in_h, in_w)
            dz = torch.empty((n, self.cin, in_h, in_w), dtype=torch.float32, device=dy.device)
            pk = self._packed("dgrad", w, g)
            src, dst = make_src(dy), make_dst(dz)
            _, _, _, asn, asc = _planes(a)
            rc = L.lib().pcuda_conv2d_dgrad_lrelu(C.byref(g), _precision, C.byref(src), pk.data_ptr(), C.byref(dst),
                                                  a.data_ptr(), asn, asc, float(slope), _stream())
            if rc == 0:
                return dz
            if rc != L.PCUDA_E_UNSUPPORTED:
                check(rc, "conv2d_dgrad_lrelu")
        return lrelu_bwd(self.dgrad(dy, w, in_h, in_w), a, slope)

    def dgrad_fold(self, dy, w, in_h, in_w, bnred=None):
        assert self.in_up
        n = dy.shape[0]
        g = self.geom(n, in_h, in_w)
        lib = L.lib()
        if _fold_dgrad and in_h % 2 == 0 and in_w % 4 == 0:
            pk = self._packed("dgrad", w, g)
            dx = torch.empty((n, self.cin, in_h // 2, in_w // 2), dtype=torch.float32, device=dy.device)
            src, dst = make_src(dy), make_dst(dx)
            a_p = m_p = i_p = r_p = None
            asn = asc = 0
            red, nt = None, 0
            if bnred is not None and _fuse_bnred:
                a, st = bnred
                nt = lib.pcuda_conv2d_dgrad_tiles(C.byref(g), _precision)
                if nt > 0:
                    _, _, _, asn, asc = _planes(a)
                    red = torch.empty((nt, self.cin, 2), dtype=torch.float32, device=dy.device)
                    a_p, m_p, i_p, r_p = a.data_ptr(), st.mean.data_ptr(), st.invstd.data_ptr(), red.data_ptr()
            rc = lib.pcuda_conv2d_dgrad_fold(C.byref(g), _precision, C.byref(src), pk.data_ptr(), C.byref(dst), a_p, asn, asc,
                                             m_p, i_p, r_p, _stream())
            if rc == 0:
                if bnred is None:
                    return dx
                return (dx, (red, nt)) if red is not None else upsample_red_only(dx, bnred)
            if rc != L.PCUDA_E_UNSUPPORTED:
                check(rc, "conv2d_dgrad_fold")
        d_up = self.dgrad(dy, w, in_h, in_w)
        return upsample2_bwd(d_up, bnred=bnred)

    def wgrad(self, x, dy, dw, db, in_h, in_w, x2=None, accumulate=True):
        xa = _as_ta(x)
        n = xa.t.shape[0]
        g = self.geom(n, in_h, in_w)
        lib = L.lib()
        ws_bytes = lib.pcuda_conv2d_wgrad_workspace_size(C.byref(g))
        ws = torch.empty(ws_bytes, dtype=torch.uint8, device=dy.device)
        _, _, _, sn, sc = _planes(dy)
        src = make_src(xa, x2)
        pend = getattr(_deferred, "jobs", None)
        if pend is not None:
            job = L.ReduceJob()
            check(lib.pcuda_conv2d_wgrad_partial(C.byref(g), _precision, C.byref(src), dy.data_ptr(), sn, sc, dw.data_ptr(),
                                                 _ptr(db), 1 if accumulate else 0, ws.data_ptr(), ws_bytes, C.byref(job),
                                                 _stream()), "conv2d_wgrad_partial")
            if job.ksplit > 0:
                if any(j.dw == job.dw for j, _ in pend):
                    flush_wgrad_reduces()
                pend.append((job, ws))
                if _batch_reduce_n >= 2 and len(pend) >= _batch_reduce_n:
                    flush_wgrad_reduces()
            return
        check(lib.pcuda_conv2d_wgrad(C.byref(g), _precision, C.byref(src), dy.data_ptr(), sn, sc, dw.data_ptr(),
                                     _ptr(db), 1 if accumulate else 0, ws.data_ptr(), ws_bytes, _stream()),
              "conv2d_wgrad")


_batch_reduce_n = int(os.environ.get("PCUDA_BATCH_REDUCE", "0") or 0)
_batch_reduce = _batch_reduce_n >= 1
_deferred = threading.local()


def flush_wgrad_reduces():
    pend = getattr(_deferred, "jobs", None)
    if not pend:
        return
    arr = (L.ReduceJob * len(pend))(*[j for j, _ in pend])
    check(L.lib().pcuda_wgrad_reduce_batch(arr, len(pend), _stream()), "wgrad_reduce_batch")
    del pend[:]


class deferred_wgrad_reduces:

    def __enter__(self):
        self.outer = getattr(_deferred, "jobs", None)
        if _batch_reduce and self.outer is None:
            _deferred.jobs = []
        return self

    def __exit__(self, *exc):
        if _batch_reduce and self.outer is None:
            try:
                if exc[0] is None:
                    flush_wgrad_reduces()
            finally:
                _deferred.jobs = None
        return False


_batch_repack = os.environ.get("PCUDA_PACK_TABLE", "1") != "0"


def repack_owner(owner):
    if not _batch_repack:
        return False
    lib = L.lib()
    ops = [op for op in _conv_ops if op.owner is owner and op._last_fwd is not None]
    if not ops:
        return False
    gen = getattr(owner, "_wgen", 0)
    key, entries = [], []
    for op in ops:
        w, g = op._last_fwd
        fhit = op._pk.get(("fwd", _precision))
        dhit = op._pk.get(("dgrad", _precision)) if op.pack_dgrad_with_fwd else None
        if fhit is None or fhit[0] != w.data_ptr() or (op.pack_dgrad_with_fwd and dhit is None):
            continue
        entries.append((op, w, g, fhit[3], None if dhit is None else dhit[3]))
# ... 5 lines not shown
    if tab is None or tab[0] != key:
        jb = lib.pcuda_conv2d_pack_job_bytes()
        chunks, blocks = [], []
        for op, w, g, fb, db in entries:
            host = C.create_string_buffer(jb * 8)
            jblk = (C.c_int * 8)()
            nj = lib.pcuda_conv2d_pack_jobs_fill(C.byref(g), _precision, w.data_ptr(), fb.data_ptr(),
                                                 None if db is None else db.data_ptr(), host, 8, jblk)
            if nj < 0:
                check(nj, "pack_jobs_fill")
            chunks.append(host.raw[:jb * nj]); blocks += list(jblk[:nj])
        dev = entries[0][1].device
        blob = torch.frombuffer(bytearray(b"".join(chunks)), dtype=torch.uint8).to(dev)
        first = torch.tensor([sum(blocks[:j]) for j in range(len(blocks))], dtype=torch.int32).to(dev)
        tab = (key, blob, first, len(blocks), sum(blocks))
        owner._pack_table = tab
    check(lib.pcuda_conv2d_pack_table(tab[1].data_ptr(), tab[2].data_ptr(), tab[3], tab[4], _stream()), "pack_table")
    for op, w, g, fb, db in entries:
        op._pk[("fwd", _precision)] = (w.data_ptr(), w._version, gen, fb)
        if db is not None:
            op._pk[("dgrad", _precision)] = (w.data_ptr(), w._version, gen, db)
    return True


class BNState:
    __slots__ = ("mean", "invstd", "scale", "shift", "count")

    @classmethod
    def empty(cls, c, count, device):
        st = cls()
        buf = torch.empty((4, c), dtype=torch.float32, device=device)
        st.mean, st.invstd, st.scale, st.shift, st.count = buf[0], buf[1], buf[2], buf[3], count
        return st


def _opt_planes(t: Optional[torch.Tensor]):
    return (None, 0, 0) if t is None else (t.data_ptr(),) + _planes(t)[3:]


def _ntiles(n, c, hw):
    nt = C.c_int(0)
    check(L.lib().pcuda_bn_stats(None, 0, 0, n, c, hw, None, C.byref(nt), None), "bn_stats(query)")
    return nt.value


def bn_finalize(partials, ntiles, count, gamma, beta, running_mean, running_var, eps=1e-5, momentum=0.1) -> BNState:
    c = partials.shape[1]
    st = BNState.empty(c, count, partials.device)
    check(L.lib().pcuda_bn_finalize(partials.data_ptr(), ntiles, c, count, _ptr(gamma), _ptr(beta), eps, momentum,
                                    _ptr(running_mean), _ptr(running_var), st.mean.data_ptr(), st.invstd.data_ptr(),
                                    st.scale.data_ptr(), st.shift.data_ptr(), _stream()), "bn_finalize")
    return st


def bn_stats(a: torch.Tensor):
    n, c, hw, sn, sc = _planes(a)
    nt = _ntiles(n, c, hw)
    partials = torch.empty((nt, c, 2), dtype=torch.float32, device=a.device)
    check(L.lib().pcuda_bn_stats(a.data_ptr(), sn, sc, n, c, hw, partials.data_ptr(), None, _stream()), "bn_stats")
    return partials, nt, n * hw


def bn_apply(a: torch.Tensor, st: BNState, relu=False, out=None, fma=False):
    n, c, hw, sn, sc = _planes(a)
    if out is None:
        out = torch.empty_like(a, memory_format=torch.contiguous_format)
    _, _, _, osn, osc = _planes(out)
    flags = (1 if relu else 0) | (2 if fma else 0)
    check(L.lib().pcuda_bn_apply(a.data_ptr(), sn, sc, st.scale.data_ptr(), st.shift.data_ptr(), flags,
                                 out.data_ptr(), osn, osc, n, c, hw, _stream()), "bn_apply")
    return out


_pn_small = os.environ.get("PCUDA_PN_SMALL", "1") != "0"


def _bn1d_ok(*ts):
    return _pn_small and all(t.dim() == 2 and t.shape[0] <= 1024 and t.stride(1) == 1 and t.shape[1] <= t.stride(0) <= 1 << 20
                             for t in ts)


def bn1d_forward(a, gamma, beta, running_mean, running_var, relu=False, eps=1e-5, momentum=0.1):
    _req(a)
    if not _bn1d_ok(a):
        return None
    b, c = a.shape
    st = BNState.empty(c, b, a.device)
    y = torch.empty((b, c), dtype=torch.float32, device=a.device)
    check(L.lib().pcuda_bn1d_fwd(a.data_ptr(), a.stride(0), b, c, _ptr(gamma), _ptr(beta), eps, momentum,
                                 _ptr(running_mean), _ptr(running_var), st.mean.data_ptr(), st.invstd.data_ptr(),
                                 st.scale.data_ptr(), st.shift.data_ptr(), 1 if relu else 0, y.data_ptr(), y.stride(0),
                                 _stream()), "bn1d_fwd")
    return st, y


def bn_backward(dy, a, st: BNState, gamma, dgamma, dbeta, dy2=None, post_relu=False, act_slope=1.0,
                accumulate=True, red=None, frozen=False):
    if dy2 is None and red is None and not frozen and _bn1d_ok(a, dy):
        _req(a); _req(dy)
        b, c = a.shape
        dz = torch.empty((b, c), dtype=torch.float32, device=a.device)
        check(L.lib().pcuda_bn1d_bwd(dy.data_ptr(), dy.stride(0), a.data_ptr(), a.stride(0), b, c, _ptr(gamma),
                                     st.mean.data_ptr(), st.invstd.data_ptr(), st.scale.data_ptr(), st.shift.data_ptr(),
                                     1 if post_relu else 0, float(act_slope), _ptr(dgamma), _ptr(dbeta),
                                     1 if accumulate else 0, dz.data_ptr(), dz.stride(0), _stream()), "bn1d_bwd")
        return dz
    n, c, hw, asn, asc = _planes(a)
    dyp, d2p = _opt_planes(dy), _opt_planes(dy2)
    lib = L.lib()
    pr = 1 if post_relu else 0
    if red is not None:
        assert dy2 is None and not post_relu

    def reduce():
        if red is not None:
            return red
        part = torch.empty((_ntiles(n, c, hw), c, 2), dtype=torch.float32, device=a.device)
        check(lib.pcuda_bn_bwd_reduce(*dyp, *d2p, a.data_ptr(), asn, asc, st.mean.data_ptr(), st.invstd.data_ptr(),
                                      st.scale.data_ptr(), st.shift.data_ptr(), pr, n, c, hw, part.data_ptr(), None,
                                      _stream()), "bn_bwd_reduce")
        return part, part.shape[0]

    def apply(coef, dz):
        check(lib.pcuda_bn_bwd_apply(*dyp, *d2p, a.data_ptr(), asn, asc, coef.data_ptr(), st.scale.data_ptr(),
                                     st.shift.data_ptr(), pr, float(act_slope), *_opt_planes(dz), n, c, hw, _stream()),
              "bn_bwd_apply")

    return _bn_backward_chain(a, n * hw, st, gamma, dgamma, dbeta, accumulate, frozen, reduce, apply)


def _bn_backward_chain(a, count, st, gamma, dgamma, dbeta, accumulate, frozen, reduce, apply):
    c = a.shape[1]
    part, ntiles = reduce()
    coef = torch.empty((c, 3), dtype=torch.float32, device=a.device)
    check(L.lib().pcuda_bn_bwd_finalize(part.data_ptr(), ntiles, c, -count if frozen else count, _ptr(gamma),
                                        st.invstd.data_ptr(), st.mean.data_ptr(), _ptr(dgamma), _ptr(dbeta),
                                        1 if accumulate else 0, coef.data_ptr(), _stream()), "bn_bwd_finalize")
    dz = torch.empty(a.shape, dtype=torch.float32, device=a.device)
    apply(coef, dz)
    return dz


def make_pooled(g, idx, h, w, g2=None):
    p = L.Pooled()
    p.g, p.g_sn, p.g_sc = _opt_planes(g)
    p.g2, p.g2_sn, p.g2_sc = _opt_planes(g2)
    assert idx.is_contiguous() and idx.dtype == torch.uint8
    p.idx, p.h, p.w = idx.data_ptr(), h, w
    return p


_fuse_pool = os.environ.get("PCUDA_FUSE_POOL_BWD", "1") != "0"
_fuse_lrelu_dgrad = os.environ.get("PCUDA_FUSE_LRELU_DGRAD", "1") != "0"


def lrelu_bwd_pooled(g, idx, a, slope, g2=None, dy=None):
    n, c, hw, asn, asc = _planes(a)
    h, w = a.shape[2], a.shape[3]
    if not _fuse_pool:
        return lrelu_bwd(maxpool2_bwd(g, idx, h, w, dy2=g2), a, slope, dy2=dy)
    dz = torch.empty(a.shape, dtype=torch.float32, device=a.device)
    pool = make_pooled(g, idx, h, w, g2)
    check(L.lib().pcuda_lrelu_bwd_pooled(C.byref(pool), *_opt_planes(dy), a.data_ptr(), asn, asc, float(slope),
                                         *_opt_planes(dz), n, c, _stream()), "lrelu_bwd_pooled")
    return dz


def bn_backward_pooled(g, idx, a, st: BNState, gamma, dgamma, dbeta, g2=None, dy=None, act_slope=1.0, accumulate=True,
                       frozen=False):
    n, c, hw, asn, asc = _planes(a)
    h, w = a.shape[2], a.shape[3]
    if not _fuse_pool:
        return bn_backward(maxpool2_bwd(g, idx, h, w, dy2=g2), a, st, gamma, dgamma, dbeta, dy2=dy, act_slope=act_slope,
                           accumulate=accumulate, frozen=frozen)
    lib = L.lib()
    dyp = _opt_planes(dy)
    pool = make_pooled(g, idx, h, w, g2)

    def reduce():
        part = torch.empty((_ntiles(n, c, hw), c, 2), dtype=torch.float32, device=a.device)
        check(lib.pcuda_bn_bwd_reduce_pooled(C.byref(pool), *dyp, a.data_ptr(), asn, asc, st.mean.data_ptr(),
                                             st.invstd.data_ptr(), n, c, part.data_ptr(), None, _stream()),
              "bn_bwd_reduce_pooled")
        return part, part.shape[0]

    def apply(coef, dz):
        check(lib.pcuda_bn_bwd_apply_pooled(C.byref(pool), *dyp, a.data_ptr(), asn, asc, coef.data_ptr(), float(act_slope),
                                            *_opt_planes(dz), n, c, _stream()), "bn_bwd_apply_pooled")

    return _bn_backward_chain(a, n * hw, st, gamma, dgamma, dbeta, accumulate, frozen, reduce, apply)


def lrelu_bwd(dy, a, slope, dy2=None):
    n, c, hw, asn, asc = _planes(a)
    dz = torch.empty(a.shape, dtype=torch.float32, device=a.device)
    check(L.lib().pcuda_lrelu_bwd(*_opt_planes(dy), *_opt_planes(dy2), a.data_ptr(), asn, asc, float(slope),
                                  *_opt_planes(dz), n, c, hw, _stream()), "lrelu_bwd")
    return dz


def channel_sum(dz, db, accumulate=True):
    n, c, hw, sn, sc = _planes(dz)
    ws = torch.empty((_ntiles(n, c, hw), c), dtype=torch.float32, device=dz.device)
    check(L.lib().pcuda_channel_sum(dz.data_ptr(), sn, sc, n, c, hw, db.data_ptr(), 1 if accumulate else 0,
                                    ws.data_ptr(), ws.numel() * 4, _stream()), "channel_sum")


def maxpool2_fwd(x):
    xa = _as_ta(x)
    n, c, _, sn, sc = _planes(xa.t)
    h, w = xa.t.shape[2], xa.t.shape[3]
    y = torch.empty((n, c, h // 2, w // 2), dtype=torch.float32, device=xa.t.device)
    idx = torch.empty((n, c, h // 2, w // 2), dtype=torch.uint8, device=xa.t.device)
    check(L.lib().pcuda_maxpool2_fwd(xa.t.data_ptr(), sn, sc, _ptr(xa.scale), _ptr(xa.shift), y.data_ptr(),
                                     y.stride(0), y.stride(1), idx.data_ptr(), n, c, h, w, _stream()), "maxpool2_fwd")
    return y, idx


def maxpool2_bwd(dy, idx, h, w, dy2=None):
    n, c, _, dsn, dsc = _planes(dy)
    dx = torch.empty((n, c, h, w), dtype=torch.float32, device=dy.device)
    check(L.lib().pcuda_maxpool2_bwd(dy.data_ptr(), dsn, dsc, *_opt_planes(dy2), idx.data_ptr(), dx.data_ptr(),
                                     dx.stride(0), dx.stride(1), 0, n, c, h, w, _stream()), "maxpool2_bwd")
    return dx


def upsample2_bwd(dy, bnred=None):
    n, c, _, dsn, dsc = _planes(dy)
    h, w = dy.shape[2] // 2, dy.shape[3] // 2
    dx = torch.empty((n, c, h, w), dtype=torch.float32, device=dy.device)
    lib = L.lib()
    if bnred is not None and _fuse_bnred:
        a, st = bnred
        _, _, _, asn, asc = _planes(a)
        red = torch.empty((_ntiles(n, c, h * w), c, 2), dtype=torch.float32, device=dy.device)
        check(lib.pcuda_upsample2_bwd_bnred(dy.data_ptr(), dsn, dsc, dx.data_ptr(), dx.stride(0), dx.stride(1), 0,
                                            a.data_ptr(), asn, asc, st.mean.data_ptr(), st.invstd.data_ptr(),
                                            red.data_ptr(), None, n, c, h, w, _stream()), "upsample2_bwd_bnred")
        return dx, (red, red.shape[0])
    check(lib.pcuda_upsample2_bwd(dy.data_ptr(), dsn, dsc, dx.data_ptr(), dx.stride(0), dx.stride(1), 0, n, c, h,
                                  w, _stream()), "upsample2_bwd")
    return (dx, None) if bnred is not None else dx


def bilinear_fwd(x, oh, ow):
    n, c, _, xsn, xsc = _planes(x)
    h, w = x.shape[2], x.shape[3]
    y = torch.empty((n, c, oh, ow), dtype=torch.float32, device=x.device)
    check(L.lib().pcuda_bilinear_fwd(x.data_ptr(), xsn, xsc, n, c, h, w, y.data_ptr(), oh, ow, _stream()), "bilinear_fwd")
    return y


def bilinear_bwd(dy, h, w):
    _req(dy)
    dy = dy.contiguous()
    n, c, oh, ow = dy.shape
    dx = torch.empty((n, c, h, w), dtype=torch.float32, device=dy.device)
    check(L.lib().pcuda_bilinear_bwd(dy.data_ptr(), n, c, oh, ow, dx.data_ptr(), dx.stride(0), dx.stride(1), h, w,
                                     _stream()), "bilinear_bwd")
    return dx


def d1_forward_direct(op, n, h, w):
    g = op.geom(n, h, w)
    return bool(L.lib().pcuda_conv2d_d1_forward_ok(C.byref(g)))


def unfold_taps(x, k, stride, pad, dil=1):
    n, c, _, xsn, xsc = _planes(x)
    h, w = x.shape[2], x.shape[3]
    oh = (h + 2 * pad - dil * (k - 1) - 1) // stride + 1
    ow = (w + 2 * pad - dil * (k - 1) - 1) // stride + 1
    u = torch.empty((n, c * k * k, oh, ow), dtype=torch.float32, device=x.device)
    check(L.lib().pcuda_unfold_taps(x.data_ptr(), xsn, xsc, n, c, h, w, k, stride, pad, dil, u.data_ptr(), oh, ow,
                                    _stream()), "unfold_taps")
    return u


def add_n(ts, out=None):
    ts = [t for t in ts if t is not None]
    for t in ts:
        _req(t)
        if not t.is_contiguous():
            raise ValueError("add_n needs contiguous tensors")
    if out is None:
        out = torch.empty_like(ts[0])
    p = [t.data_ptr() for t in ts] + [None] * (4 - len(ts))
    check(L.lib().pcuda_add4(p[0], p[1], p[2], p[3], out.data_ptr(), out.numel(), _stream()), "add4")
    return out


def mul(a, b):
    _req(a); _req(b)
    a, b = a.contiguous(), b.contiguous()
    y = torch.empty_like(a)
    check(L.lib().pcuda_mul(a.data_ptr(), b.data_ptr(), y.data_ptr(), a.numel(), _stream()), "mul")
    return y


def _mode(m):
    return ACT_SIGMOID if m in (ACT_SIGMOID, "sigmoid") else ACT_SOFTMAX


def entropy_fwd(logits, mode="sigmoid", norm=1.0, want_prob=False):
    _req(logits)
    logits = logits.contiguous()
    n, c = logits.shape[:2]
    hw = logits.numel() // (n * c)
    ent = torch.empty_like(logits)
# ... 1074 lines not shown
```

pointcloududa_amd/networks/unet.py:

```python
from __future__ import annotations

import os

import numpy as np
import torch
from torch import nn

from .. import kernels as K
from ..kernels import TA, ConvOp
from ._holders import (BatchNorm2d, Conv2d, LeakyReLU, Linear, Marker, collect, ensure_grad)

SLOPE = 0.01




class _SegEngine:

    def __init__(self, filters, in_channels, n_block, depth, n_class, pointnet, fc_inch, extpn=False, batchnorm=True,
                 feature_dis=False, parts=None, head_ch=None, num_points=300):
        f = filters
        self.f, self.cin, self.nb, self.depth, self.ncls, self.pointnet, self.fc_inch = \
            f, in_channels, n_block, depth, n_class, pointnet, fc_inch
        self.extpn = bool(extpn and pointnet)
        self.bn = bool(batchnorm)
        self.c2 = ".3" if self.bn else ".2"
        self.feature_dis = bool(feature_dis)
        self.head_ch = 512 * f // 32 if head_ch is None else head_ch
        self.npts = num_points
        self.after_deep_grads = None
        parts = ("encoder", "bottleneck", "pointNet", "decoder", "classifier") if parts is None else parts
        ops = {}
        if "encoder" in parts:
            for i in range(n_block):
                co = f * 2 ** i
                ci = in_channels if i == 0 else f * 2 ** (i - 1)
                blk = "encoder.encoder%d" % (i + 1)
                ops[blk + ".0"] = ConvOp(ci, co, 3, pad=1)
                ops[blk + self.c2] = ConvOp(co, co, 3, pad=1)
                if i > 0:
                    ops["encoder.conv1_%d.0" % (i + 1)] = ConvOp(ci * 3, co, 1)
        if "bottleneck" in parts:
            co, ci = f * 2 ** n_block, f * 2 ** (n_block - 1)
            for j in range(depth):
                d = 2 ** j
                ops["bottleneck.bottleneck%d.0" % (j + 1)] = ConvOp(ci, co, 3, pad=d, dil=d)
                ci = co
        if pointnet and "pointNet" in parts:
            ch = self.head_ch
            if self.extpn:
                ops["pointNet.conv1"] = ConvOp(ch, 2 * ch, 3, pad=1)
                ops["pointNet.conv2"] = ConvOp(2 * ch, ch, 3, pad=1)
            ops["pointNet.final_conv"] = ConvOp(ch, num_points, 6)
        if "decoder" in parts:
            for i in range(n_block):
                co = f * 2 ** i
                ops["decoder.decoder1_%d.1" % (i + 1)] = ConvOp(2 * co, co, 3, pad=1, in_up=True)
                blk = "decoder.decoder2_%d" % (i + 1)
                ops[blk + ".0"] = ConvOp(2 * co, co, 3, pad=1)
                ops[blk + self.c2] = ConvOp(co, co, 3, pad=1)
        if "classifier" in parts:
            ops["classifier"] = ConvOp(f, n_class, 1)
            if self.feature_dis:
                ops["classifier2"] = ConvOp(512, n_class, 1)
        self.ops = ops

    @staticmethod
    def _bn(P, name, partials, nt, count, training, c_dev):
        if training:
            return K.bn_finalize(partials, nt, count, P[name + ".weight"], P[name + ".bias"],
                                 P[name + ".running_mean"], P[name + ".running_var"])
        st = K.BNState()
        inv = torch.rsqrt(P[name + ".running_var"] + 1e-5)
        st.mean, st.invstd = P[name + ".running_mean"], inv
        st.scale = (P[name + ".weight"] * inv).contiguous()
        st.shift = (P[name + ".bias"] - P[name + ".running_mean"] * st.scale).contiguous()
        st.count = count
        return st

    def _dc_fwd(self, P, blk, x, x2, h, w, training, S):
        n = (x.t if isinstance(x, TA) else x).shape[0]
        if not self.bn:
            a0, _, _ = self.ops[blk + ".0"].forward(x, P[blk + ".0.weight"], P[blk + ".0.bias"], SLOPE, h, w, x2=x2)
            a1, _, _ = self.ops[blk + ".2"].forward(a0, P[blk + ".2.weight"], P[blk + ".2.bias"], SLOPE, h, w)
            S[blk] = (x, x2, a0, None, a1, None)
            return a1
        a0, part, nt = self.ops[blk + ".0"].forward(x, P[blk + ".0.weight"], P[blk + ".0.bias"], SLOPE, h, w, x2=x2,
                                                    want_stats=training)
        st0 = self._bn(P, blk + ".2", part, nt, n * h * w, training, a0.device)
        a1, part, nt = self.ops[blk + ".3"].forward(TA(a0, st0.scale, st0.shift), P[blk + ".3.weight"],
                                                    P[blk + ".3.bias"], SLOPE, h, w, want_stats=training)
        st1 = self._bn(P, blk + ".5", part, nt, n * h * w, training, a1.device)
        S[blk] = (x, x2, a0, st0, a1, st1)
        return TA(a1, st1.scale, st1.shift)

    def _dc_bwd(self, P, G, blk, dy, dy2, h, w, S, need_dx, red=None, pooled=None):
        x, x2, a0, st0, a1, st1 = S[blk]
        if not self.bn:
            if pooled is not None:
                dz1 = K.lrelu_bwd_pooled(pooled[0], pooled[2], a1, SLOPE, g2=pooled[1], dy=dy2)
            else:
                dz1 = K.lrelu_bwd(dy, a1, SLOPE, dy2=dy2)
            if G(blk + ".2.weight") is not None:
                self.ops[blk + ".2"].wgrad(a0, dz1, G(blk + ".2.weight"), G(blk + ".2.bias"), h, w)
            dz0 = K.lrelu_bwd(self.ops[blk + ".2"].dgrad(dz1, P[blk + ".2.weight"], h, w), a0, SLOPE)
            return self._dc_bwd_first(P, G, blk, x, x2, dz0, h, w, need_dx)
        frozen = not S["training"]
        if pooled is not None:
            dz1 = K.bn_backward_pooled(pooled[0], pooled[2], a1, st1, P[blk + ".5.weight"], G(blk + ".5.weight"),
                                       G(blk + ".5.bias"), g2=pooled[1], dy=dy2, act_slope=SLOPE, frozen=frozen)
        else:
            dz1 = K.bn_backward(dy, a1, st1, P[blk + ".5.weight"], G(blk + ".5.weight"), G(blk + ".5.bias"), dy2=dy2,
                                act_slope=SLOPE, red=red if dy2 is None else None, frozen=frozen)
        if G(blk + ".3.weight") is not None:
            self.ops[blk + ".3"].wgrad(TA(a0, st0.scale, st0.shift), dz1, G(blk + ".3.weight"), G(blk + ".3.bias"), h, w)
        d_y0, red = self.ops[blk + ".3"].dgrad(dz1, P[blk + ".3.weight"], h, w, bnred=(a0, st0))
        dz0 = K.bn_backward(d_y0, a0, st0, P[blk + ".2.weight"], G(blk + ".2.weight"), G(blk + ".2.bias"),
                            act_slope=SLOPE, red=red, frozen=frozen)
        return self._dc_bwd_first(P, G, blk, x, x2, dz0, h, w, need_dx)

    def _dc_bwd_first(self, P, G, blk, x, x2, dz0, h, w, need_dx):
        if G(blk + ".0.weight") is not None:
            self.ops[blk + ".0"].wgrad(x, dz0, G(blk + ".0.weight"), G(blk + ".0.bias"), h, w, x2=x2)
        if not need_dx:
            return None, None
        op0 = self.ops[blk + ".0"]
        n = dz0.shape[0]
        if x2 is None:
            return op0.dgrad(dz0, P[blk + ".0.weight"], h, w), None
        c1 = (x.t if isinstance(x, TA) else x).shape[1]
        dx1 = torch.empty((n, c1, h, w), dtype=torch.float32, device=dz0.device)
        dx2 = torch.empty((n, op0.cin - c1, h, w), dtype=torch.float32, device=dz0.device)
        op0.dgrad(dz0, P[blk + ".0.weight"], h, w, dx=dx1, dx2=dx2)
        return dx1, dx2

    @staticmethod
    def new_state(P, training):
        return {"wants": {k for k, p in P.items() if p.requires_grad}, "training": training}

    @staticmethod
    def grad_of(P, S):
        wants = S["wants"]

        def G(name):
            return ensure_grad(P[name]) if name in wants else None
        return G

    def fwd_encoder(self, P, x, training, S):
        _, _, h, w = x.shape
        cur, res, skips = x, None, []
        for i in range(self.nb):
            y = self._dc_fwd(P, "encoder.encoder%d" % (i + 1), cur, None, h, w, training, S)
            skips.append(y)
            if i > 0:
                c1 = "encoder.conv1_%d.0" % (i + 1)
                t, _, _ = self.ops[c1].forward(y, P[c1 + ".weight"], P[c1 + ".bias"], SLOPE, h, w, x2=res)
                S[c1] = (y, res, t)
                pooled, idx = K.maxpool2_fwd(t)
            else:
                pooled, idx = K.maxpool2_fwd(y)
            S["pool%d" % i] = idx
            res = cur = pooled
            h, w = h // 2, w // 2
        return cur, skips

    def fwd_bottleneck(self, P, x, h, w, S):
        outs, o = [], x
        for j in range(self.depth):
            name = "bottleneck.bottleneck%d.0" % (j + 1)
            S[name] = o
            o, _, _ = self.ops[name].forward(o, P[name + ".weight"], P[name + ".bias"], SLOPE, h, w)
            outs.append(o)
        bsum = outs[0]
        for k0 in range(1, len(outs), 3):
            bsum = K.add_n([bsum] + outs[k0:k0 + 3])
        S["bott_outs"] = outs
        return bsum

    def fwd_head(self, P, x, h, w, S):
        n = x.shape[0]
        hin, ext_acts = x, []
        if self.extpn:
            for nm in ("pointNet.conv1", "pointNet.conv2"):
                o, _, _ = self.ops[nm].forward(hin, P[nm + ".weight"], P[nm + ".bias"], SLOPE, h, w)
                ext_acts.append((nm, hin, o))
                hin = o
        S["head_ext"] = ext_acts
        hc, _, _ = self.ops["pointNet.final_conv"].forward(hin, P["pointNet.final_conv.weight"],
                                                           P["pointNet.final_conv.bias"], SLOPE, h, w)
        flat = hc.view(n * self.npts, -1)
        if flat.shape[1] != self.fc_inch:
            raise ValueError("fc_inch=%d does not match the %dx%d head output" % (self.fc_inch, h - 5, w - 5))
        verts = K.linear_fwd(flat, P["pointNet.final_fc.weight"], P["pointNet.final_fc.bias"]).view(n, self.npts, 3)
        S["head"] = (hin, hc, flat)
        return verts

    def fwd_decoder(self, P, x, skips, h, w, training, S):
        prev, ph, pw = x, h, w
        for i in reversed(range(self.nb)):
            up = "decoder.decoder1_%d.1" % (i + 1)
            oh, ow = 2 * ph, 2 * pw
            S[up] = prev
            u, _, _ = self.ops[up].forward(prev, P[up + ".weight"], P[up + ".bias"], 1.0, oh, ow)
            prev = self._dc_fwd(P, "decoder.decoder2_%d" % (i + 1), skips[i], u, oh, ow, training, S)
            ph, pw = oh, ow
        return prev

    def forward(self, P, x, training):
        n, _, H, W = x.shape
        nb = self.nb
        if H % (1 << nb) or W % (1 << nb):
            raise ValueError("input size must be divisible by %d" % (1 << nb))
        S = self.new_state(P, training)
        S["hw"], S["n"] = (H, W), n
        cur, skips = self.fwd_encoder(P, x, training, S)
        h, w = H >> nb, W >> nb
        bsum = self.fwd_bottleneck(P, cur, h, w, S)
        verts = self.fwd_head(P, bsum, h, w, S) if self.pointnet else None
        out2 = None
        if self.feature_dis:
            S["bsum"] = bsum
            out2, _, _ = self.ops["classifier2"].forward(bsum, P["classifier2.weight"], P["classifier2.bias"], 1.0, h, w)
        S["out2"] = out2
        prev = self.fwd_decoder(P, bsum, skips, h, w, training, S)
        S["cls_in"] = prev
        logits, _, _ = self.ops["classifier"].forward(prev, P["classifier.weight"], P["classifier.bias"], 1.0, H, W)
        return logits, verts, S

    @staticmethod
    def _bn_of(S, i):
        blk = S["decoder.decoder2_%d" % (i + 1)]
        return blk[4], blk[5]

    def bwd_decoder(self, P, G, S, d_cur, red, H, W, fused):
        nb = self.nb
        d_skips = [None] * nb
        for i in range(nb):
            oh, ow = H >> i, W >> i
            d_skips[i], d_u = self._dc_bwd(P, G, "decoder.decoder2_%d" % (i + 1), d_cur, None, oh, ow, S, True, red=red)
            up = "decoder.decoder1_%d.1" % (i + 1)
            if G(up + ".weight") is not None:
                self.ops[up].wgrad(S[up], d_u, G(up + ".weight"), G(up + ".bias"), oh, ow)
            if fused and i + 1 < nb and self.bn:
                d_cur, red = self.ops[up].dgrad_fold(d_u, P[up + ".weight"], oh, ow, bnred=self._bn_of(S, i + 1))
            else:
                d_cur, red = self.ops[up].dgrad_fold(d_u, P[up + ".weight"], oh, ow), None
        return d_cur, d_skips

    def bwd_head(self, P, G, S, d_verts, d_x, h, w):
        hin, hc, flat = S["head"]
        d_v = d_verts.contiguous().view(-1, 3)
        if G("pointNet.final_fc.weight") is not None:
            K.linear_bwd_w(d_v, flat, G("pointNet.final_fc.weight"), G("pointNet.final_fc.bias"))
        d_hc = K.linear_bwd_x(d_v, P["pointNet.final_fc.weight"]).view(hc.shape)
        dzc = K.lrelu_bwd(d_hc, hc, SLOPE)
        op, op_name = self.ops["pointNet.final_conv"], "pointNet.final_conv"
        if G("pointNet.final_conv.weight") is not None:
            op.wgrad(hin, dzc, G("pointNet.final_conv.weight"), G("pointNet.final_conv.bias"), h, w)
        for nm, xin, o in reversed(S["head_ext"]):
            d_o = op.dgrad(dzc, P[op_name + ".weight"], h, w)
            dzc = K.lrelu_bwd(d_o, o, SLOPE)
            op, op_name = self.ops[nm], nm
            if G(nm + ".weight") is not None:
                op.wgrad(xin, dzc, G(nm + ".weight"), G(nm + ".bias"), h, w)
        if d_x is None:
            return op.dgrad(dzc, P[op_name + ".weight"], h, w)
        op.dgrad(dzc, P[op_name + ".weight"], h, w, dx=d_x, accumulate=True)
        return d_x

    def bwd_bottleneck(self, P, G, S, d_bsum, h, w, need_dx=True):
        outs, g_next = S["bott_outs"], None
        for j in reversed(range(self.depth)):
            name = "bottleneck.bottleneck%d.0" % (j + 1)
            dz = K.lrelu_bwd(d_bsum, outs[j], SLOPE, dy2=g_next)
            if G(name + ".weight") is not None:
                self.ops[name].wgrad(S[name], dz, G(name + ".weight"), G(name + ".bias"), h, w)
            if j > 0 or need_dx:
                g_next = self.ops[name].dgrad(dz, P[name + ".weight"], h, w)
        return g_next

    def bwd_encoder(self, P, G, S, d_out, d_skips, H, W, need_dx):
        dA, dB = d_out, None
        for i in reversed(range(self.nb)):
            hi, wi = H >> i, W >> i
            idx = S["pool%d" % i]
            if i > 0:
                c1 = "encoder.conv1_%d.0" % (i + 1)
                y, res_prev, t = S[c1]
                dzc = K.lrelu_bwd_pooled(dA, idx, t, SLOPE, g2=dB)
                if G(c1 + ".weight") is not None:
                    self.ops[c1].wgrad(y, dzc, G(c1 + ".weight"), G(c1 + ".bias"), hi, wi, x2=res_prev)
                d_y = torch.empty((y.t if isinstance(y, TA) else y).shape, dtype=torch.float32, device=dzc.device)
                dB = torch.empty(res_prev.shape, dtype=torch.float32, device=dzc.device)
                self.ops[c1].dgrad(dzc, P[c1 + ".weight"], hi, wi, dx=d_y, dx2=dB)
                pooled = None
            else:
                d_y, pooled, dB = None, (dA, dB, idx), None
            dA, _ = self._dc_bwd(P, G, "encoder.encoder%d" % (i + 1), d_y, d_skips[i], hi, wi, S, i > 0 or need_dx,
                                 pooled=pooled)
        return dA

    def backward(self, P, S, d_logits, d_verts, need_dx, d_out2=None):
        G = self.grad_of(P, S)
        nb, (H, W) = self.nb, S["hw"]
        d_skips = [None] * nb
        d_bsum = None
        if d_logits is not None:
            d_logits = d_logits.contiguous()
            if G("classifier.weight") is not None:
                self.ops["classifier"].wgrad(S["cls_in"], d_logits, G("classifier.weight"), G("classifier.bias"), H, W)
            if self.bn:
                d_cur, red = self.ops["classifier"].dgrad(d_logits, P["classifier.weight"], H, W, bnred=self._bn_of(S, 0))
            else:
                d_cur, red = self.ops["classifier"].dgrad(d_logits, P["classifier.weight"], H, W), None
            d_bsum, d_skips = self.bwd_decoder(P, G, S, d_cur, red, H, W, fused=True)
        h, w = H >> nb, W >> nb
        if self.feature_dis and d_out2 is not None:
            d_out2 = d_out2.contiguous()
            op2 = self.ops["classifier2"]
            if G("classifier2.weight") is not None:
                op2.wgrad(S["bsum"], d_out2, G("classifier2.weight"), G("classifier2.bias"), h, w)
            if d_bsum is None:
                d_bsum = op2.dgrad(d_out2, P["classifier2.weight"], h, w)
            else:
                op2.dgrad(d_out2, P["classifier2.weight"], h, w, dx=d_bsum, accumulate=True)
        if self.pointnet and d_verts is not None:
            d_bsum = self.bwd_head(P, G, S, d_verts, d_bsum, h, w)
        if d_bsum is None:
            return None
        g_next = self.bwd_bottleneck(P, G, S, d_bsum, h, w)
        cb = self.after_deep_grads
        if cb is not None:
            K.flush_wgrad_reduces()
            cb()
        return self.bwd_encoder(P, G, S, g_next, d_skips, H, W, need_dx)


class _SegFn(torch.autograd.Function):
    @staticmethod
    def forward(ctx, module, x, *params):
        if not x.is_cuda:
            raise RuntimeError("Segmentation_model_Point runs on HIP devices only (no CPU fallback)")
        x = x.contiguous().float()
        P = module._tensor_dict()
        logits, verts, S = module._engine.forward(P, x, module.training)
        if module.training:
            module._bump_batches_tracked()
        ctx.module, ctx.S, ctx.P = module, S, P
        if getattr(module, "_keep_state", False):
            module._last_S = S
        ctx.set_materialize_grads(False)
        out2 = S.get("out2")
        ctx.layout = (verts is not None, out2 is not None)
        outs = [logits] + ([verts] if verts is not None else []) + ([out2] if out2 is not None else [])
        return outs[0] if len(outs) == 1 else tuple(outs)

    @staticmethod
    def backward(ctx, d_logits, *rest):
        rest = list(rest)
        d_verts = rest.pop(0) if ctx.layout[0] else None
        d_out2 = rest.pop(0) if ctx.layout[1] else None
        with K.deferred_wgrad_reduces():
            dx = ctx.module._engine.backward(ctx.P, ctx.S, d_logits, d_verts, ctx.needs_input_grad[1], d_out2=d_out2)
        ctx.S = None
        return (None, dx) + (None,) * (len(ctx.needs_input_grad) - 2)


class _StageFn(torch.autograd.Function):

    @staticmethod
    def forward(ctx, module, n_in, *tensors):
        eng, P = module._stage_engine()
        S = eng.new_state(P, module.training)
        xs = [t.contiguous().float() for t in tensors[:n_in]]
        outs = module._stage_fwd(eng, P, xs, S)
        if module.training:
            for k, b in module.named_buffers():
                if k.endswith("num_batches_tracked"):
                    b.add_(1)
        if getattr(module, "_keep_state", False):
            module._last_S = S
        ctx.module, ctx.eng, ctx.P, ctx.S, ctx.n_in = module, eng, P, S, n_in
        ctx.set_materialize_grads(False)
        return tuple(outs)

    @staticmethod
    def backward(ctx, *grads):
        need = ctx.needs_input_grad[2:2 + ctx.n_in]
        dxs = [None] * ctx.n_in
        if any(g is not None for g in grads):
            with K.deferred_wgrad_reduces():
                dxs = ctx.module._stage_bwd(ctx.eng, ctx.P, ctx.S, [g if g is None else g.contiguous() for g in grads],
                                            need)
        ctx.S = ctx.P = None
        return (None, None) + tuple(d if n else None for d, n in zip(dxs, need)) + \
            (None,) * (len(ctx.needs_input_grad) - 2 - ctx.n_in)


def _hip_only(module, *xs):
    for x in xs:
        if not (torch.is_tensor(x) and x.is_cuda):
            raise RuntimeError("%s runs on HIP devices only (no CPU fallback)" % type(module).__name__)


def _check_shape(module, what, x, shape):
    if tuple(x.shape) != tuple(shape):
        raise ValueError("%s: %s has shape %s, expected %s" % (type(module).__name__, what, tuple(x.shape), tuple(shape)))


def _materialise(y):
    return K.bn_apply(y.t, _Affine(y.scale, y.shift), fma=True) if isinstance(y, TA) else y


class _Affine:
    __slots__ = ("scale", "shift")

    def __init__(self, scale, shift):
        self.scale, self.shift = scale, shift


class _Stage(nn.Module):
    _name = ""

    def _attach(self, host):
        object.__setattr__(self, "_host", host)

    def _stage_engine(self):
        host = self.__dict__.get("_host")
        if host is not None and getattr(host, self._name, None) is self:
            eng = host._engine
        else:
            eng = self.__dict__.get("_own_engine")
            if eng is None:
                eng = self._make_engine()
                for op in eng.ops.values():
                    op.owner = self
                self._own_engine = eng
        pre = self._name + "."
        P = {pre + k: v for k, v in self.named_parameters()}
        P.update({pre + k: v for k, v in self.named_buffers()})
        return eng, P


class Encoder(_Stage):
    _name = "encoder"

    def __init__(self, filters=32, in_channels=3, n_block=4, kernel_size=(3, 3), batch_norm=True, padding='same'):
        super().__init__()
        self.filter = filters
        pad = kernel_size[0] // 2 if padding == 'same' else 0
        for i in range(n_block):
            out_ch = filters * 2 ** i
            in_ch = in_channels if i == 0 else filters * 2 ** (i - 1)
            model = [Conv2d(in_ch, out_ch, kernel_size, padding=pad), LeakyReLU(inplace=True)]
            if batch_norm:
                model += [BatchNorm2d(out_ch)]
            model += [Conv2d(out_ch, out_ch, kernel_size, padding=pad), LeakyReLU(inplace=True)]
            if batch_norm:
                model += [BatchNorm2d(out_ch)]
            self.add_module('encoder%d' % (i + 1), nn.Sequential(*model))
            self.add_module('conv1_%d' % (i + 1), nn.Sequential(Conv2d(in_ch * 3, out_ch, 1), LeakyReLU(inplace=True)))
        self._cfg = (in_channels, n_block, batch_norm, tuple(kernel_size) == (3, 3) and padding == 'same')

    def _make_engine(self):
        cin, nb, bn, _ = self._cfg
        return _SegEngine(self.filter, cin, nb, 0, 0, False, 0, batchnorm=bn, parts=("encoder",))

    def forward(self, x):
        cin, nb, _, std = self._cfg
        if not std:
            raise NotImplementedError("Encoder: only kernel_size=(3, 3), padding='same' (the reference's defaults) run")
        _hip_only(self, x)
        if x.dim() != 4 or x.shape[1] != cin or x.shape[2] % (1 << nb) or x.shape[3] % (1 << nb):
            raise ValueError("Encoder: input must be [n, %d, h, w] with h and w divisible by %d, got %s"
                             % (cin, 1 << nb, tuple(x.shape)))
        out = _StageFn.apply(self, 1, x, *self.parameters())
        return out[0], list(out[1:])

    def _stage_fwd(self, eng, P, xs, S):
        S["hw"] = tuple(xs[0].shape[2:])
        cur, skips = eng.fwd_encoder(P, xs[0], S["training"], S)
        return [cur] + [_materialise(y) for y in skips]

    def _stage_bwd(self, eng, P, S, grads, need):
        d_out, d_skips = grads[0], list(grads[1:])
        if d_out is None:
            idx = S["pool%d" % (eng.nb - 1)]
            d_out = torch.zeros(idx.shape, dtype=torch.float32, device=idx.device)
        H, W = S["hw"]
        return [eng.bwd_encoder(P, eng.grad_of(P, S), S, d_out, d_skips, H, W, need[0])]


class Bottleneck(_Stage):
    _name = "bottleneck"

    def __init__(self, filters=32, n_block=4, depth=4, kernel_size=(3, 3)):
        super().__init__()
        out_ch, in_ch = filters * 2 ** n_block, filters * 2 ** (n_block - 1)
        for i in range(depth):
            d = 2 ** i
            self.add_module('bottleneck%d' % (i + 1), nn.Sequential(
                Conv2d(in_ch, out_ch, kernel_size, padding=d, dilation=d), LeakyReLU(inplace=True)))
            if i == 0:
                in_ch = out_ch
        self._cfg = (filters, n_block, depth, tuple(kernel_size) == (3, 3))

    def _make_engine(self):
        f, nb, depth, _ = self._cfg
        return _SegEngine(f, 0, nb, depth, 0, False, 0, parts=("bottleneck",))

    def forward(self, x):
        f, nb, depth, std = self._cfg
        if not std:
            raise NotImplementedError("Bottleneck: only kernel_size=(3, 3) (the reference's default) runs")
        _hip_only(self, x)
        if depth < 1:
            raise ValueError("Bottleneck: depth must be at least 1")
        if x.dim() != 4 or x.shape[1] != f * 2 ** (nb - 1):
            raise ValueError("Bottleneck: input must be [n, %d, h, w], got %s" % (f * 2 ** (nb - 1), tuple(x.shape)))
        return _StageFn.apply(self, 1, x, *self.parameters())[0]

    def _stage_fwd(self, eng, P, xs, S):
        S["hw"] = tuple(xs[0].shape[2:])
        return [eng.fwd_bottleneck(P, xs[0], S["hw"][0], S["hw"][1], S)]

    def _stage_bwd(self, eng, P, S, grads, need):
        h, w = S["hw"]
# ... 188 lines not shown
```

Baseline: 781.2 img/s.

## Fuse 1x1 encoder conv with 2x2 maxpool and gate LReLU backward on pooled activations

Adds a dedicated 1x1 MFMA conv kernel that applies bias and LeakyReLU, then writes the 2x2 max-pooled output and argmax indices directly, so the full-resolution activation is no longer materialised in training. The backward LReLU-through-pool kernel now reads the pooled activation instead of the full-resolution one to decide the slope. This is meant to cut activation write/read traffic and a separate maxpool launch in the UNet encoder. It adds a new kernel with LDS-resident weights, one wave per EU and a software pipeline, which may be slower than the existing igemm path for some shapes. It also relies on the pooled value's sign matching the selected element's sign, which holds because the max is the selected element.

Result: no change. 782.4 img/s, median of 3 (+0.2%).

```diff
diff --git a/include/pcuda_hip.h b/include/pcuda_hip.h
--- a/include/pcuda_hip.h
+++ b/include/pcuda_hip.h
@@ -77,6 +77,9 @@
 int pcuda_conv2d_forward(const pcuda_conv_geom* g, int prec, const pcuda_src* x, const void* packed_w,
                          const float* bias, float slope, const pcuda_dst* y, float* bn_partials,
                          pcuda_stream_t s);
+int pcuda_conv2d_fwd_pool(const pcuda_conv_geom* g, int prec, const pcuda_src* x, const void* packed_w, const float* bias,
+                          float slope, float* pooled, long long pooled_sn, long long pooled_sc, uint8_t* idx,
+                          const pcuda_dst* t, pcuda_stream_t s);
 int pcuda_conv2d_dgrad(const pcuda_conv_geom* g, int prec, const pcuda_src* dy, const void* packed_w_dgrad,
                        const pcuda_dst* dx, int accumulate, pcuda_stream_t s);
 int pcuda_conv2d_dgrad_tiles(const pcuda_conv_geom* g, int prec);
@@ -157,6 +160,8 @@
 int pcuda_lrelu_bwd_pooled(const pcuda_pooled* pool, const float* dy, long long dy_sn, long long dy_sc, const float* a,
                            long long a_sn, long long a_sc, float slope, float* dz, long long dz_sn, long long dz_sc, int n,
                            int c, pcuda_stream_t s);
+int pcuda_lrelu_bwd_pooled_act(const pcuda_pooled* pool, const float* pooled_act, long long act_sn, long long act_sc,
+                               float slope, float* dz, long long dz_sn, long long dz_sc, int n, int c, pcuda_stream_t s);
 int pcuda_upsample2_bwd(const float* dy, long long dy_sn, long long dy_sc, float* dx, long long dx_sn,
                         long long dx_sc, int accumulate, int n, int c, int h, int w, pcuda_stream_t s);
 int pcuda_upsample2_bwd_bnred(const float* dy, long long dy_sn, long long dy_sc, float* dx, long long dx_sn,
diff --git a/pointcloududa_amd/_lib.py b/pointcloududa_amd/_lib.py
--- a/pointcloududa_amd/_lib.py
+++ b/pointcloududa_amd/_lib.py
@@ -65,6 +65,7 @@
     "pcuda_conv2d_pack_table": (i32, [vp, vp, i32, i32, vp]),
     "pcuda_conv2d_fwd_tiles": (i32, [C.POINTER(ConvGeom), i32]),
     "pcuda_conv2d_forward": (i32, [C.POINTER(ConvGeom), i32, C.POINTER(Src), vp, vp, f32, C.POINTER(Dst), vp, vp]),
+    "pcuda_conv2d_fwd_pool": (i32, [C.POINTER(ConvGeom), i32, C.POINTER(Src), vp, vp, f32, vp, i64, i64, vp, C.POINTER(Dst), vp]),
     "pcuda_conv2d_d1_forward_ok": (i32, [C.POINTER(ConvGeom)]),
     "pcuda_conv2d_dgrad": (i32, [C.POINTER(ConvGeom), i32, C.POINTER(Src), vp, C.POINTER(Dst), i32, vp]),
     "pcuda_conv2d_dgrad_tiles": (i32, [C.POINTER(ConvGeom), i32]),
@@ -92,6 +93,7 @@
     "pcuda_bn_bwd_reduce_pooled": (i32, [C.POINTER(Pooled), vp, i64, i64, vp, i64, i64, vp, vp, i32, i32, vp, C.POINTER(i32), vp]),
     "pcuda_bn_bwd_apply_pooled": (i32, [C.POINTER(Pooled), vp, i64, i64, vp, i64, i64, vp, f32, vp, i64, i64, i32, i32, vp]),
     "pcuda_lrelu_bwd_pooled": (i32, [C.POINTER(Pooled), vp, i64, i64, vp, i64, i64, f32, vp, i64, i64, i32, i32, vp]),
+    "pcuda_lrelu_bwd_pooled_act": (i32, [C.POINTER(Pooled), vp, i64, i64, f32, vp, i64, i64, i32, i32, vp]),
     "pcuda_upsample2_bwd": (i32, [vp, i64, i64, vp, i64, i64, i32, i32, i32, i32, i32, vp]),
     "pcuda_upsample2_bwd_bnred": (i32, [vp, i64, i64, vp, i64, i64, i32, vp, i64, i64, vp, vp, vp, C.POINTER(i32), i32, i32,
                                         i32, i32, vp]),
diff --git a/pointcloududa_amd/csrc/conv_host.h b/pointcloududa_amd/csrc/conv_host.h
--- a/pointcloududa_amd/csrc/conv_host.h
+++ b/pointcloududa_amd/csrc/conv_host.h
@@ -166,6 +166,12 @@
 bool rs_map_ok(int n, int h, int w);
 int rs_tiles(int n, int h, int w);
 int rs_try_launch(const IgemmParams& p, int prec, const TapSet& taps, hipStream_t s, int* rc);
+
+struct Pw1Pool {
+  float* pooled; long long sn, sc;
+  unsigned char* idx;
+};
+int pw1_try_launch(const IgemmParams& p, int prec, const TapSet& taps, hipStream_t s, int* rc, const Pw1Pool* pool = nullptr);
 
 static inline size_t packed_elems(int rows, int red, int ntaps, int prec) {
   const int co_tile = 32 * ig_co_blks(rows);
diff --git a/pointcloududa_amd/csrc/conv_igemm.hip b/pointcloududa_amd/csrc/conv_igemm.hip
--- a/pointcloududa_amd/csrc/conv_igemm.hip
+++ b/pointcloududa_amd/csrc/conv_igemm.hip
@@ -311,6 +311,7 @@
     int rc;
     if (ap_image && prec == PCUDA_PREC_BF16X3 && ap_try_launch(p, taps, ap_image, s, &rc)) return rc;
     if (p.cin == 32 && p.cout == 32 && rs_try_launch(p, prec, taps, s, &rc)) return rc;
+    if (taps.n == 1 && pw1_try_launch(p, prec, taps, s, &rc)) return rc;
   }
   const bool x3 = prec == PCUDA_PREC_BF16X3;
   const int co_blks = ig_co_blks(p.cout);
@@ -464,6 +465,24 @@
   return im ? (const unsigned char*)packed + im->off : nullptr;
 }
 
+static IgemmParams fwd_params(const pcuda_conv_geom* g, const pcuda_src* x, const pcuda_dst* y, const void* packed_w,
+                              const PackedLayout& L, const float* bias, float slope) {
+  IgemmParams p;
+  memset(&p, 0, sizeof(p));
+  p.x = *x; p.cin = g->cin;
+  p.in_h = g->in_h; p.in_w = g->in_w; p.in_shift = g->in_up ? 1 : 0; p.in_row = g->in_w >> p.in_shift;
+  if (y) p.y = *y;
+  p.cout = g->cout; p.out_w = g->out_w;
+  p.lh = g->out_h; p.lw = g->out_w;
+  p.oy_mul = p.ox_mul = 1; p.oy_off = p.ox_off = 0;
+  p.in_step = g->stride;
+  p.wpack = (const uint16_t*)image_ptr(packed_w, &L.img[0]);
+  p.w_lo_off = 0;
+  p.bias = bias; p.slope = slope; p.accumulate = 0; p.stats = nullptr;
+  p.n = g->n;
+  return p;
+}
+
 extern "C" int pcuda_conv2d_forward(const pcuda_conv_geom* g, int prec, const pcuda_src* x, const void* packed_w,
                                     const float* bias, float slope, const pcuda_dst* y, float* bn_partials,
                                     pcuda_stream_t s) {
@@ -480,20 +499,27 @@
   }
   PackedLayout L;
   packed_layout(g, prec, SIDE_FWD, &L);
-  IgemmParams p;
-  memset(&p, 0, sizeof(p));
-  p.x = *x; p.cin = g->cin;
-  p.in_h = g->in_h; p.in_w = g->in_w; p.in_shift = g->in_up ? 1 : 0; p.in_row = g->in_w >> p.in_shift;
-  p.y = *y; p.cout = g->cout; p.out_w = g->out_w;
-  p.lh = g->out_h; p.lw = g->out_w;
-  p.oy_mul = p.ox_mul = 1; p.oy_off = p.ox_off = 0;
-  p.in_step = g->stride;
-  p.wpack = (const uint16_t*)image_ptr(packed_w, &L.img[0]);
-  p.w_lo_off = 0;
-  p.bias = bias; p.slope = slope; p.accumulate = 0; p.stats = bn_partials;
-  p.n = g->n;
+  IgemmParams p = fwd_params(g, x, y, packed_w, L, bias, slope);
+  p.stats = bn_partials;
   const ConvRoute route = bn_partials ? conv_route(g, prec, SIDE_FWD, false) : ConvRoute{ROUTE_IGEMM, -1};
   return launch_igemm(p, prec, L.img[0].taps, (hipStream_t)s, image_ptr(packed_w, L.ap()), &route);
+}
+
+extern "C" int pcuda_conv2d_fwd_pool(const pcuda_conv_geom* g, int prec, const pcuda_src* x, const void* packed_w,
+                                     const float* bias, float slope, float* pooled, long long pooled_sn, long long pooled_sc,
+                                     uint8_t* idx, const pcuda_dst* t, pcuda_stream_t s) {
+  if (!geom_ok(g)) PCUDA_FAIL(PCUDA_E_BADARG, "conv2d_fwd_pool: inconsistent geometry");
+  if (!src_ok(x, g->cin) || (t && !dst_ok(t, g->cout)) || !packed_w || !pooled || !idx) PCUDA_FAIL(PCUDA_E_BADARG, "conv2d_fwd_pool: bad tensors");
+  if (prec != PCUDA_PREC_BF16X3 && prec != PCUDA_PREC_BF16) PCUDA_FAIL(PCUDA_E_BADARG, "conv2d_fwd_pool: bad precision");
+  if (g->k != 1 || g->stride != 1 || g->pad != 0 || g->in_up || (g->in_h & 1) || (g->in_w & 1) || direct_fwd_tiles(g))
+    PCUDA_FAIL(PCUDA_E_UNSUPPORTED, "conv2d_fwd_pool: stride-1 1x1 MFMA layers on even maps only");
+  PackedLayout L;
+  packed_layout(g, prec, SIDE_FWD, &L);
+  IgemmParams p = fwd_params(g, x, t, packed_w, L, bias, slope);
+  const Pw1Pool pool = {pooled, pooled_sn, pooled_sc, idx};
+  int rc;
+  if (pw1_try_launch(p, prec, L.img[0].taps, (hipStream_t)s, &rc, &pool)) return rc;
+  PCUDA_FAIL(PCUDA_E_UNSUPPORTED, "conv2d_fwd_pool: this geometry does not run on the 1x1 kernel");
 }
 
 static int dgrad_impl(const pcuda_conv_geom* g, int prec, const pcuda_src* dy, const void* packed_w_dgrad,
diff --git a/pointcloududa_amd/csrc/conv_pw1.hip b/pointcloududa_amd/csrc/conv_pw1.hip
--- /dev/null
+++ b/pointcloududa_amd/csrc/conv_pw1.hip
@@ -0,0 +1,452 @@
+#include <algorithm>
+#include <stdlib.h>
+#include <type_traits>
+#include <utility>
+
+#include "conv_igemm.h"
+#include "conv_device.h"
+#include "conv_host.h"
+#include "variants.h"
+
+namespace {
+
+#ifndef PW1_DEPTH
+#define PW1_DEPTH 4
+#endif
+constexpr int PW1_D = PW1_DEPTH;
+constexpr int PW1_RB = 4;
+
+struct Pw1Params {
+  pcuda_src x; int red;
+  pcuda_dst y; int rows;
+  int n, h, w, hw;
+  const unsigned char* wimg;
+  int wbytes, nchunks, co_shift;
+  const float* bias; float slope;
+  float* pooled; long long p_sn, p_sc; unsigned char* idx;
+  int bpi, bx;
+  int items, nrb, npass;
+};
+
+struct Pw1It { int item, pass, chunk; };
+
+template <class F, int... I>
+__device__ __forceinline__ void pw1_static_for(std::integer_sequence<int, I...>, F&& f) {
+  (f(std::integral_constant<int, I>{}), ...);
+}
+
+template <bool X3> struct Pw1Raw {
+  f32x4 v[4];
+  int c;
+  bool ok, aff;
+};
+
+template <bool X3, bool POOL, bool WRES>
+__global__ __launch_bounds__(256, 1) __attribute__((amdgpu_waves_per_eu(1, 1))) void conv_pw1_kernel(const Pw1Params p) {
+  extern __shared__ __attribute__((aligned(16))) unsigned char smem[];
+  constexpr int REC = IgRec<X3>::BYTES;
+  constexpr int SLOT = X3 ? 32 * REC : 4096;
+  const int tid = threadIdx.x, lane = tid & 63, r = lane & 31, h = lane >> 5;
+  const int w = __builtin_amdgcn_readfirstlane(tid >> 6);
+  const int lq = lane & 7, lg = (lane >> 3) & 3, cbl = 8 * lg + 4 * h;
+
+  const int xc1 = __builtin_amdgcn_readfirstlane(p.x.c1);
+  unsigned char* const wl = smem;
+  unsigned char* const ring = smem + (WRES ? p.wbytes : 0) + w * (2 * SLOT);
+  float* const sbias = (float*)(smem + (WRES ? p.wbytes : 0) + 4 * (2 * SLOT));
+  float* const sscale = sbias + p.nrb * 32;
+  float* const sshift = sscale + p.nchunks * 32;
+
+  if (WRES) {
+    const int nvec = p.wbytes >> 4;
+    for (int i = tid; i < nvec; i += 256) *(uint4*)(wl + i * 16) = *(const uint4*)(p.wimg + (size_t)i * 16);
+  }
+  for (int i = tid; i < p.nrb * 32; i += 256) sbias[i] = p.bias ? p.bias[min(i, p.rows - 1)] : 0.f;
+  for (int i = tid; i < p.nchunks * 32; i += 256) {
+    const int c = min(i, p.red - 1);
+    const bool first = c < xc1;
+    const float* scp = first ? p.x.scale1 : p.x.scale2;
+    const float* shp = first ? p.x.shift1 : p.x.shift2;
+    const int cc = first ? c : c - xc1;
+    sscale[i] = scp ? scp[cc] : 1.f;
+    sshift[i] = scp ? shp[cc] : 0.f;
+  }
+  __syncthreads();
+
+  const int nx = min(8, (int)gridDim.x);
+  const int xcd = blockIdx.x % nx, wslot = (blockIdx.x / nx) * 4 + w;
+  const int gx = ((int)gridDim.x - xcd + nx - 1) / nx;
+  const int lo = (int)((long long)p.items * xcd / nx), hi = (int)((long long)p.items * (xcd + 1) / nx);
+  const int stride = gx * 4;
+
+  const __amdgpu_buffer_rsrc_t wrs = __builtin_amdgcn_make_buffer_rsrc((void*)p.wimg, 0, p.wbytes, 0x00020000);
+  const unsigned wlane = (unsigned)(r * REC + h * 16);
+
+  auto adv = [&](Pw1It& it) {
+    if (++it.chunk == p.nchunks) {
+      it.chunk = 0;
+      if (++it.pass == p.npass) { it.pass = 0; it.item += stride; }
+    }
+  };
+  auto decode = [&](int item, int& img, unsigned& poff, bool& pv) {
+    const int itc = min(item, p.items - 1);
+    img = __builtin_amdgcn_readfirstlane(itc / p.bpi);
+    const int blk = itc - img * p.bpi;
+    if (POOL) {
+      const int by = blk / p.bx, bxk = blk - by * p.bx;
+      const int x = 16 * bxk + 4 * (lq & 3);
+      poff = (unsigned)((2 * by + (lq >> 2)) * p.w + x);
+      pv = (item < hi) & (x < p.w);
+    } else {
+      poff = (unsigned)(blk * 32 + 4 * lq);
+      pv = (item < hi) & ((int)poff < p.hw);
+    }
+  };
+  auto issue = [&](Pw1Raw<X3>& q, const Pw1It& it) {
+    int img; unsigned poff; bool pv;
+    decode(__builtin_amdgcn_readfirstlane(it.item), img, poff, pv);
+    const int c0 = __builtin_amdgcn_readfirstlane(it.chunk) * 32;
+    const bool first = c0 < xc1;
+    const float* base = first ? p.x.p1 + (long long)img * p.x.sn1 : p.x.p2 + (long long)img * p.x.sn2;
+    const int csrc = first ? min(xc1, p.red) : p.red - xc1;
+    const int cl = (first ? c0 : c0 - xc1) + cbl;
+    const unsigned plane = (unsigned)(first ? p.x.sc1 : p.x.sc2) * 4u;
+    const __amdgpu_buffer_rsrc_t rs = __builtin_amdgcn_make_buffer_rsrc((void*)base, 0, (int)(csrc * plane), 0x00020000);
+    q.ok = pv & (cl < csrc);
+    const unsigned voff = q.ok ? (unsigned)cl * plane + poff * 4u : IG_OOB;
+#pragma unroll
+    for (int e = 0; e < 4; ++e)
+      q.v[e] = __builtin_bit_cast(f32x4, __builtin_amdgcn_raw_buffer_load_b128(rs, voff, e * plane, 0));
+    q.aff = (first ? p.x.scale1 : p.x.scale2) != nullptr;
+    q.c = c0 + cbl;
+  };
+  auto convert = [&](const Pw1Raw<X3>& q, int s) {
+    unsigned char* const dst = ring + s * SLOT + (4 * lq) * REC + cbl * 2;
+    f32x4 sc = {1.f, 1.f, 1.f, 1.f}, sh = {0.f, 0.f, 0.f, 0.f};
+    if (q.aff) { sc = *(const f32x4*)(sscale + q.c); sh = *(const f32x4*)(sshift + q.c); }
+#pragma unroll
+    for (int j = 0; j < 4; ++j) {
+      float a[4];
+#pragma unroll
+      for (int e = 0; e < 4; ++e) {
+        a[e] = q.v[e][j];
+        if (q.aff) a[e] = fmaf(a[e], sc[e], sh[e]);
+        a[e] = q.ok ? a[e] : 0.f;
+      }
+      uint2 vh, vl;
+      if (X3) {
+        split2(a[0], a[1], vh.x, vl.x); split2(a[2], a[3], vh.y, vl.y);
+        *(uint2*)(dst + j * REC + IG_LO_OFF) = vl;
+      } else {
+        vh.x = pack_bf16x2(a[0], a[1]); vh.y = pack_bf16x2(a[2], a[3]);
+      }
+      *(uint2*)(dst + j * REC) = vh;
+    }
+  };
+
+  f32x16 acc[PW1_RB];
+  Pw1Raw<X3> raw[PW1_D];
+  Pw1It ci = {__builtin_amdgcn_readfirstlane(lo + wslot), 0, 0}, ii = ci;
+  pw1_static_for(std::make_integer_sequence<int, PW1_D>{}, [&](auto DD) { issue(raw[decltype(DD)::value], ii); adv(ii); });
+  convert(raw[0], 0);
+  issue(raw[0], ii); adv(ii);
+
+  while (ci.item < hi) {
+    pw1_static_for(std::make_integer_sequence<int, PW1_D>{}, [&](auto DD) {
+      constexpr int d = decltype(DD)::value;
+      constexpr int dn = (d + 1) % PW1_D;
+      convert(raw[dn], (d + 1) & 1);
+      issue(raw[dn], ii); adv(ii);
+
+      const int cvalid = min(32, p.red - ci.chunk * 32);
+      const int nks = cvalid > 16 ? 2 : 1;
+      const int nrbp = min(PW1_RB, p.nrb - ci.pass * PW1_RB);
+      if (ci.chunk == 0) {
+#pragma unroll
+        for (int rb = 0; rb < PW1_RB; ++rb)
+#pragma unroll
+          for (int i = 0; i < 16; ++i) acc[rb][i] = 0.f;
+      }
+      const unsigned char* const xs = ring + (d & 1) * SLOT + r * REC + h * 16;
+#pragma unroll
+      for (int ks = 0; ks < 2; ++ks) {
+        if (ks < nks) {
+          const bf16x8 bh = lds_frag(xs + ks * 32);
+          bf16x8 bl = bh;
+          if (X3) bl = lds_frag(xs + IG_LO_OFF + ks * 32);
+#pragma unroll
+          for (int rb = 0; rb < PW1_RB; ++rb) {
+            if (rb < nrbp) {
+              const int grb = ci.pass * PW1_RB + rb;
+              const int cot = grb >> p.co_shift, cb = grb - (cot << p.co_shift);
+              const unsigned wo = (unsigned)(((cot * p.nchunks + ci.chunk) << p.co_shift) + cb) * (32u * REC) + ks * 32;
+              bf16x8 ah, al;
+              if (WRES) {
+                ah = lds_frag(wl + wo + wlane);
+                al = ah;
+                if (X3) al = lds_frag(wl + wo + wlane + IG_LO_OFF);
+              } else {
+                ah = __builtin_bit_cast(bf16x8, __builtin_amdgcn_raw_buffer_load_b128(wrs, wlane, wo, 0));
+                al = ah;
+                if (X3) al = __builtin_bit_cast(bf16x8, __builtin_amdgcn_raw_buffer_load_b128(wrs, wlane, wo + IG_LO_OFF, 0));
+              }
+              if (X3) {
+                acc[rb] = __builtin_amdgcn_mfma_f32_32x32x16_bf16(al, bh, acc[rb], 0, 0, 0);
+                acc[rb] = __builtin_amdgcn_mfma_f32_32x32x16_bf16(ah, bl, acc[rb], 0, 0, 0);
+              }
+              acc[rb] = __builtin_amdgcn_mfma_f32_32x32x16_bf16(ah, bh, acc[rb], 0, 0, 0);
+            }
+          }
+        }
+      }
+
+      if (ci.chunk == p.nchunks - 1) {
+        int img; unsigned poff; bool pv;
+        decode(ci.item, img, poff, pv);
+        float* const tsc = (float*)(ring + (d & 1) * SLOT);
+        const int q = lane & 7, cs = lane >> 3;
+        const int c1 = min(p.y.c1, p.rows);
+        const bool have_y = !POOL || p.y.p1 != nullptr;
+#pragma unroll
+        for (int rb = 0; rb < PW1_RB; ++rb) {
+          if (rb < nrbp) {
+            const int co0 = (ci.pass * PW1_RB + rb) * 32;
+#pragma unroll
+            for (int i = 0; i < 16; ++i) tsc[((i & 3) + 8 * (i >> 2) + 4 * h) * 32 + r] = acc[rb][i];
+            __builtin_amdgcn_wave_barrier();
+            if (have_y) {
+              const bool first = co0 < c1;
+              float* const yb = first ? p.y.p1 + (long long)img * p.y.sn1 : p.y.p2 + (long long)img * p.y.sn2;
+              const unsigned plane = (unsigned)(first ? p.y.sc1 : p.y.sc2) * 4u;
+              const int cdst = first ? c1 : p.rows - c1, cl0 = first ? co0 : co0 - c1;
+              const __amdgpu_buffer_rsrc_t ys = __builtin_amdgcn_make_buffer_rsrc((void*)yb, 0, (int)(cdst * plane), 0x00020000);
+#pragma unroll
+              for (int it = 0; it < 4; ++it) {
+                const int cl = it * 8 + cs;
+                f32x4 v = *(const f32x4*)(tsc + cl * 32 + 4 * q);
+                const float b = sbias[co0 + cl];
+#pragma unroll
+                for (int e = 0; e < 4; ++e) {
+                  const float t = v[e] + b;
+                  v[e] = t > 0.f ? t : t * p.slope;
+                }
+                const bool ok = pv & (cl0 + cl < cdst);
+                const unsigned vo = ok ? (unsigned)(cl0 + cl) * plane + poff * 4u : IG_OOB;
+                __builtin_amdgcn_raw_buffer_store_b128(__builtin_bit_cast(u32x4, v), ys, vo, 0, 0);
+              }
+            }
+            if (POOL) {
+              const int wq = lane & 3, cs16 = lane >> 2;
+              const int blk = min(ci.item, p.items - 1) - img * p.bpi;
+              const int by = blk / p.bx, bxk = blk - by * p.bx;
+              const int x = 16 * bxk + 4 * wq;
+              const bool wv = (ci.item < hi) & (x < p.w);
+              const unsigned ooff = (unsigned)(by * (p.w >> 1) + (x >> 1));
+              const unsigned ohw = (unsigned)((p.h >> 1) * (p.w >> 1));
+              const __amdgpu_buffer_rsrc_t ps = __builtin_amdgcn_make_buffer_rsrc(
+                  (void*)(p.pooled + (long long)img * p.p_sn), 0, (int)((unsigned)p.rows * (unsigned)p.p_sc * 4u), 0x00020000);
+              const __amdgpu_buffer_rsrc_t is = __builtin_amdgcn_make_buffer_rsrc(
+                  (void*)(p.idx + (long long)img * p.rows * ohw), 0, (int)((unsigned)p.rows * ohw), 0x00020000);
+#pragma unroll
+              for (int it = 0; it < 2; ++it) {
+                const int cl = it * 16 + cs16, co = co0 + cl;
+                f32x4 a0 = *(const f32x4*)(tsc + cl * 32 + 4 * wq);
+                f32x4 a1 = *(const f32x4*)(tsc + cl * 32 + 16 + 4 * wq);
+                const float b = sbias[co];
+#pragma unroll
+                for (int e = 0; e < 4; ++e) {
+                  const float t0 = a0[e] + b, t1 = a1[e] + b;
+                  a0[e] = t0 > 0.f ? t0 : t0 * p.slope;
+                  a1[e] = t1 > 0.f ? t1 : t1 * p.slope;
+                }
+                float m[2];
+                unsigned k[2];
+#pragma unroll
+                for (int u = 0; u < 2; ++u) {
+                  m[u] = a0[2 * u]; k[u] = 0;
+                  if (a0[2 * u + 1] > m[u]) { m[u] = a0[2 * u + 1]; k[u] = 1; }
+                  if (a1[2 * u] > m[u]) { m[u] = a1[2 * u]; k[u] = 2; }
+                  if (a1[2 * u + 1] > m[u]) { m[u] = a1[2 * u + 1]; k[u] = 3; }
+                }
+                const bool ok = wv & (co < p.rows);
+                const unsigned po = ok ? ((unsigned)co * (unsigned)p.p_sc + ooff) * 4u : IG_OOB;
+                const unsigned io = ok ? (unsigned)co * ohw + ooff : IG_OOB;
+                __builtin_amdgcn_raw_buffer_store_b32(__builtin_bit_cast(unsigned, m[0]), ps, po, 0, 0);
+                __builtin_amdgcn_raw_buffer_store_b32(__builtin_bit_cast(unsigned, m[1]), ps, po, 4, 0);
+                __builtin_amdgcn_raw_buffer_store_b16((unsigned short)(k[0] | (k[1] << 8)), is, io, 0, 0);
+              }
+            }
+            __builtin_amdgcn_wave_barrier();
+          }
+        }
+      }
+      adv(ci);
+    });
+  }
+}
+
+int pw1_mode() {
+  static const int m = env_knob("PCUDA_PW1", 1);
+  return m;
+}
+
+int pw1_cus() {
+  static int cus = 0;
+  if (!cus) {
+    int d = 0; hipDeviceProp_t prop;
+    cus = (hipGetDevice(&d) == hipSuccess && hipGetDeviceProperties(&prop, d) == hipSuccess) ? prop.multiProcessorCount : 256;
+  }
+  return cus;
+}
+
+template <bool X3, bool POOL, bool WRES>
+int pw1_launch_t(const Pw1Params& pp, int grid, size_t lds, hipStream_t s) {
+  static DeviceOnce once;
+  if (const unsigned long long bit = once.pending()) {
+    if (hipFuncSetAttribute((const void*)conv_pw1_kernel<X3, POOL, WRES>, hipFuncAttributeMaxDynamicSharedMemorySize, LDS_HARD) != hipSuccess)
+      PCUDA_FAIL(PCUDA_E_LAUNCH, "conv_pw1_kernel: cannot opt in to %d bytes of LDS", LDS_HARD);
+    once.mark(bit);
+  }
+  hipLaunchKernelGGL((conv_pw1_kernel<X3, POOL, WRES>), dim3(grid), dim3(256), lds, s, pp);
+  PCUDA_CHECK_LAUNCH("conv_pw1_kernel");
+  return PCUDA_OK;
+}
+
+}
+
+int pw1_try_launch(const IgemmParams& p, int prec, const TapSet& taps, hipStream_t s, int* rc, const Pw1Pool* pool) {
+  if (!pw1_mode() || taps.n != 1 || taps.dy[0] || taps.dx[0]) return 0;
+  if (env_knob("PCUDA_PW1_SKIP", 0)) return 0;
+  const bool walk_ok = env_knob("PCUDA_PW1_WALK", 0) != 0;
+  if (prec != PCUDA_PREC_BF16X3 && prec != PCUDA_PREC_BF16) return 0;
+  if (p.in_step != 1 || p.in_shift || p.pair || p.mask_a || p.fold || p.stats || p.red_a || p.accumulate) return 0;
+  if (p.oy_mul != 1 || p.ox_mul != 1 || p.oy_off || p.ox_off) return 0;
+  if (p.lh != p.in_h || p.lw != p.in_w || p.out_w != p.in_w || p.in_row != p.in_w) return 0;
+  const long long hw = (long long)p.in_h * p.in_w;
+  if ((hw & 3) || hw >= (1ll << 24) || (p.cin & 7) || p.cin < 32 || p.n < 1) return 0;
+  const bool x3 = prec == PCUDA_PREC_BF16X3;
+  const int xc1 = p.x.c1 < p.cin ? p.x.c1 : p.cin;
+  if (xc1 < p.cin && (xc1 & 31)) return 0;
+  if (!fast_src_ok(&p.x, p.cin) || !aligned16(p.x.p1, p.x.sn1, p.x.sc1)) return 0;
+  if (xc1 < p.cin && !aligned16(p.x.p2, p.x.sn2, p.x.sc2)) return 0;
+  const bool have_y = p.y.p1 != nullptr;
+  if (!have_y && !pool) return 0;
+  if (have_y) {
+    const int yc1 = p.y.c1 < p.cout ? p.y.c1 : p.cout;
+    if (yc1 < p.cout && (yc1 & 31)) return 0;
+    if (!fast_dst_ok(&p.y, p.cout) || !aligned16(p.y.p1, p.y.sn1, p.y.sc1)) return 0;
+    if (yc1 < p.cout && !aligned16(p.y.p2, p.y.sn2, p.y.sc2)) return 0;
+  }
+  if (pool) {
+    if ((p.in_h & 1) || (p.in_w & 3) || !pool->pooled || !pool->idx) return 0;
+    if ((((uintptr_t)pool->pooled) & 7) || (pool->sn & 1) || (pool->sc & 1)) return 0;
+    if ((long long)(p.cout + 1) * pool->sc * 4 >= (1ll << 30) || (long long)p.cout * (hw / 4) >= (1ll << 30)) return 0;
+  }
+  const int rec = ig_rec_bytes(x3), slot = x3 ? 32 * rec : 4096;
+  const int co_blks = ig_co_blks(p.cout), co_tile = 32 * co_blks;
+  Pw1Params pp;
+  memset(&pp, 0, sizeof(pp));
+  pp.x = p.x; pp.red = p.cin;
+  pp.y = p.y; pp.rows = p.cout;
+  if (!have_y) memset(&pp.y, 0, sizeof(pp.y));
+  pp.n = p.n; pp.h = p.in_h; pp.w = p.in_w; pp.hw = (int)hw;
+  pp.wimg = (const unsigned char*)p.wpack;
+  pp.nchunks = cdiv(p.cin, 32);
+  pp.co_shift = co_blks == 2 ? 1 : 0;
+  const long long wbytes = (long long)cdiv(p.cout, co_tile) * pp.nchunks * co_tile * rec;
+  if (wbytes >= (1ll << 30)) return 0;
+  pp.wbytes = (int)wbytes;
+  pp.bias = p.bias; pp.slope = p.slope;
+  pp.nrb = cdiv(p.cout, 32); pp.npass = cdiv(pp.nrb, PW1_RB);
+  if (pool) {
+    pp.pooled = pool->pooled; pp.p_sn = pool->sn; pp.p_sc = pool->sc; pp.idx = pool->idx;
+    pp.bx = cdiv(p.in_w, 16); pp.bpi = (p.in_h / 2) * pp.bx;
+  } else {
+    pp.bx = 1; pp.bpi = cdiv(hw, 32);
+  }
+  const long long items = (long long)p.n * pp.bpi;
+  if (items >= (1ll << 28)) return 0;
+  pp.items = (int)items;
+  const size_t tail = 4 * (size_t)(2 * slot) + ((size_t)pp.nrb + 2 * (size_t)pp.nchunks) * 32 * sizeof(float);
+  if (tail > (size_t)LDS_HARD / 2) return 0;
+  const bool wres = (size_t)wbytes + tail <= (size_t)LDS_HARD;
+  if (!wres && !walk_ok) return 0;
+  const size_t lds = (wres ? (size_t)wbytes : 0) + tail;
+  const int grid = (int)std::min<long long>((items + 3) / 4, pw1_cus());
+  const double flops = 2.0 * p.n * (double)hw * p.cout * (double)p.cin;
+  char tag[160];
+  snprintf(tag, sizeof(tag), "pw1 n%d red%d rows%d %dx%d pool%d t%d wres%d lds%zu", p.n, p.cin, p.cout, p.in_h, p.in_w, pool ? 1 : 0,
+           have_y ? 1 : 0, wres ? 1 : 0, lds);
+  ProfScope prof(PCUDA_FAM_CONV_FWD, flops, s, tag);
+#define PW1_GO(X, P, W) *rc = pw1_launch_t<X, P, W>(pp, grid, lds, s)
+  if (x3) {
+    if (pool) { if (wres) PW1_GO(true, true, true); else PW1_GO(true, true, false); }
+    else { if (wres) PW1_GO(true, false, true); else PW1_GO(true, false, false); }
+  } else {
+    if (pool) { if (wres) PW1_GO(false, true, true); else PW1_GO(false, true, false); }
+    else { if (wres) PW1_GO(false, false, true); else PW1_GO(false, false, false); }
+  }
+#undef PW1_GO
+  note_kernel(pool ? (have_y ? "conv_pw1+pool+t" : "conv_pw1+pool") : "conv_pw1");
+  return 1;
+}
+
+namespace {
+constexpr int PG_QUADS = 1024;
+__global__ __launch_bounds__(256) void lrelu_bwd_poolgate_kernel(const float* __restrict__ g, long long g_sn, long long g_sc,
+                                                                 const float* __restrict__ g2, long long g2_sn, long long g2_sc,
+                                                                 const uint8_t* __restrict__ idx, const float* __restrict__ act,
+                                                                 long long a_sn, long long a_sc, float slope, float* __restrict__ dz,
+                                                                 long long dz_sn, long long dz_sc, int c, int h, int w) {
+  const int ch = blockIdx.y, n = blockIdx.z;
+  const int wq = w >> 2, ow = w >> 1, total = h * wq;
+  const long long ohw = (long long)(h >> 1) * ow;
+  const float* pg = g + n * g_sn + ch * g_sc;
+  const float* pg2 = g2 ? g2 + n * g2_sn + ch * g2_sc : nullptr;
+  const float* pa = act + n * a_sn + ch * a_sc;
+  const uint8_t* pi = idx + ((long long)n * c + ch) * ohw;
+  float* pz = dz + n * dz_sn + ch * dz_sc;
+  const int q1 = min(total, ((int)blockIdx.x + 1) * PG_QUADS);
+  for (int q = blockIdx.x * PG_QUADS + threadIdx.x; q < q1; q += 256) {
+    const int y = q / wq, xq = q - y * wq;
+    const long long o = (long long)(y >> 1) * ow + 2 * xq;
+    float2 gv = *(const float2*)(pg + o);
+    if (pg2) { const float2 t = *(const float2*)(pg2 + o); gv.x += t.x; gv.y += t.y; }
+    const float2 av = *(const float2*)(pa + o);
+    const unsigned short kk = *(const unsigned short*)(pi + o);
+    const int k0 = kk & 0xff, k1 = kk >> 8, krow = (y & 1) * 2;
+    f32x4 out;
+    out[0] = k0 == krow ? gv.x : 0.f;
+    out[1] = k0 == krow + 1 ? gv.x : 0.f;
+    out[2] = k1 == krow ? gv.y : 0.f;
+    out[3] = k1 == krow + 1 ? gv.y : 0.f;
+    out[0] = av.x > 0.f ? out[0] : out[0] * slope;
+    out[1] = av.x > 0.f ? out[1] : out[1] * slope;
+    out[2] = av.y > 0.f ? out[2] : out[2] * slope;
+    out[3] = av.y > 0.f ? out[3] : out[3] * slope;
+    *(f32x4*)(pz + (long long)y * w + 4 * xq) = out;
+    PCUDA_KEEP(pg + o); PCUDA_KEEP(pg2); PCUDA_KEEP(pa + o); PCUDA_KEEP(pi + o);
+  }
+}
+}
+
+extern "C" int pcuda_lrelu_bwd_pooled_act(const pcuda_pooled* pool, const float* pooled_act, long long act_sn, long long act_sc,
+                                          float slope, float* dz, long long dz_sn, long long dz_sc, int n, int c,
+                                          pcuda_stream_t s) {
+  if (!pool || !pool->g || !pool->idx || !pooled_act || !dz || n <= 0 || c <= 0 || n > 65535 || c > 65535 || pool->h <= 0 ||
+      pool->w <= 0 || (pool->h & 1) || (pool->w & 1))
+    PCUDA_FAIL(PCUDA_E_BADARG, "lrelu_bwd_pooled_act: bad arguments (even plane, g, idx, the pooled activation and dz required)");
+  auto al8 = [](const void* q, long long sn, long long sc) { return q == nullptr || ((((uintptr_t)q) & 7) == 0 && ((sn | sc) & 1) == 0); };
+  const long long ohw = (long long)(pool->h >> 1) * (pool->w >> 1);
+  if ((pool->w & 3) || !al8(pool->g, pool->g_sn, pool->g_sc) || !al8(pool->g2, pool->g2_sn, pool->g2_sc) ||
+      !al8(pooled_act, act_sn, act_sc) || !aligned16(dz, dz_sn, dz_sc) || (ohw & 1) || (long long)pool->h * pool->w >= (1ll << 30))
+    PCUDA_FAIL(PCUDA_E_UNSUPPORTED, "lrelu_bwd_pooled_act: rows of 4k pixels, 8-byte aligned pooled planes, 16-byte aligned dz");
+  const long long hw = (long long)pool->h * pool->w;
+  ProfScope prof(PCUDA_FAM_POINTWISE, (4.0 + (pool->g2 ? 2.5 : 1.5)) * n * c * (double)hw, (hipStream_t)s);
+  const int quads = (int)(hw >> 2);
+  hipLaunchKernelGGL(lrelu_bwd_poolgate_kernel, dim3((unsigned)cdiv(quads, PG_QUADS), (unsigned)c, (unsigned)n), dim3(256), 0,
+                     (hipStream_t)s, pool->g, pool->g_sn, pool->g_sc, pool->g2, pool->g2_sn, pool->g2_sc, pool->idx, pooled_act,
+                     act_sn, act_sc, slope, dz, dz_sn, dz_sc, c, pool->h, pool->w);
+  PCUDA_CHECK_LAUNCH("lrelu_bwd_poolgate_kernel");
+  return PCUDA_OK;
+}
diff --git a/pointcloududa_amd/kernels.py b/pointcloududa_amd/kernels.py
--- a/pointcloududa_amd/kernels.py
+++ b/pointcloududa_amd/kernels.py
@@ -224,6 +224,26 @@
             return out, partials, nt
         check(rc, "conv2d_forward")
         return out, partials, nt
+
+    def forward_pool(self, x, w, b, slope, in_h, in_w, x2=None, want_t=False):
+        if not _fuse_fwd_pool:
+            return None
+        xa = _as_ta(x)
+        n = xa.t.shape[0]
+        g = self.geom(n, in_h, in_w)
+        pk = self._packed("fwd", w, g)
+        dev = w.device
+        pooled = torch.empty((n, self.cout, in_h // 2, in_w // 2), dtype=torch.float32, device=dev)
+        idx = torch.empty((n, self.cout, in_h // 2, in_w // 2), dtype=torch.uint8, device=dev)
+        t = torch.empty((n, self.cout, in_h, in_w), dtype=torch.float32, device=dev) if want_t else None
+        src = make_src(xa, x2)
+        dst = C.byref(make_dst(t)) if want_t else None
+        rc = L.lib().pcuda_conv2d_fwd_pool(C.byref(g), _precision, C.byref(src), pk.data_ptr(), _ptr(b), float(slope),
+                                           pooled.data_ptr(), pooled.stride(0), pooled.stride(1), idx.data_ptr(), dst, _stream())
+        if rc == L.PCUDA_E_UNSUPPORTED:
+            return None
+        check(rc, "conv2d_fwd_pool")
+        return pooled, idx, t
 
     def dgrad(self, dy, w, in_h, in_w, dx=None, dx2=None, accumulate=False, bnred=None):
         n = dy.shape[0]
@@ -535,9 +555,20 @@
 
 _fuse_pool = os.environ.get("PCUDA_FUSE_POOL_BWD", "1") != "0"
 _fuse_lrelu_dgrad = os.environ.get("PCUDA_FUSE_LRELU_DGRAD", "1") != "0"
-
-
-def lrelu_bwd_pooled(g, idx, a, slope, g2=None, dy=None):
+_fuse_fwd_pool = _fuse_pool and os.environ.get("PCUDA_FUSE_POOL", "1") != "0"
+
+
+def lrelu_bwd_pooled(g, idx, a, slope, g2=None, dy=None, pooled=None):
+    if pooled is not None:
+        if a is not None or dy is not None:
+            raise ValueError("lrelu_bwd_pooled: pooled= replaces a and takes no full-resolution addend")
+        n, c, oh, ow = pooled.shape
+        _, _, _, asn, asc = _planes(pooled)
+        dz = torch.empty((n, c, 2 * oh, 2 * ow), dtype=torch.float32, device=pooled.device)
+        pool = make_pooled(g, idx, 2 * oh, 2 * ow, g2)
+        check(L.lib().pcuda_lrelu_bwd_pooled_act(C.byref(pool), pooled.data_ptr(), asn, asc, float(slope), *_opt_planes(dz),
+                                                 n, c, _stream()), "lrelu_bwd_pooled_act")
+        return dz
     n, c, hw, asn, asc = _planes(a)
     h, w = a.shape[2], a.shape[3]
     if not _fuse_pool:
diff --git a/pointcloududa_amd/networks/unet.py b/pointcloududa_amd/networks/unet.py
--- a/pointcloududa_amd/networks/unet.py
+++ b/pointcloududa_amd/networks/unet.py
@@ -154,9 +154,15 @@
             skips.append(y)
             if i > 0:
                 c1 = "encoder.conv1_%d.0" % (i + 1)
-                t, _, _ = self.ops[c1].forward(y, P[c1 + ".weight"], P[c1 + ".bias"], SLOPE, h, w, x2=res)
-                S[c1] = (y, res, t)
-                pooled, idx = K.maxpool2_fwd(t)
+                fused = self.ops[c1].forward_pool(y, P[c1 + ".weight"], P[c1 + ".bias"], SLOPE, h, w, x2=res,
+                                                  want_t=getattr(self, "keep_acts", False))
+                if fused is not None:
+                    pooled, idx, t = fused
+                    S[c1] = (y, res, t, pooled)
+                else:
+                    t, _, _ = self.ops[c1].forward(y, P[c1 + ".weight"], P[c1 + ".bias"], SLOPE, h, w, x2=res)
+                    pooled, idx = K.maxpool2_fwd(t)
+                    S[c1] = (y, res, t, None)
             else:
                 pooled, idx = K.maxpool2_fwd(y)
             S["pool%d" % i] = idx
@@ -286,8 +292,8 @@
             idx = S["pool%d" % i]
             if i > 0:
                 c1 = "encoder.conv1_%d.0" % (i + 1)
-                y, res_prev, t = S[c1]
-                dzc = K.lrelu_bwd_pooled(dA, idx, t, SLOPE, g2=dB)
+                y, res_prev, t, t_pooled = S[c1]
+                dzc = K.lrelu_bwd_pooled(dA, idx, None if t_pooled is not None else t, SLOPE, g2=dB, pooled=t_pooled)
                 if G(c1 + ".weight") is not None:
                     self.ops[c1].wgrad(y, dzc, G(c1 + ".weight"), G(c1 + ".bias"), hi, wi, x2=res_prev)
                 d_y = torch.empty((y.t if isinstance(y, TA) else y).shape, dtype=torch.float32, device=dzc.device)
@@ -343,6 +349,7 @@
             raise RuntimeError("Segmentation_model_Point runs on HIP devices only (no CPU fallback)")
         x = x.contiguous().float()
         P = module._tensor_dict()
+        module._engine.keep_acts = getattr(module, "_keep_state", False)
         logits, verts, S = module._engine.forward(P, x, module.training)
         if module.training:
             module._bump_batches_tracked()
@@ -373,6 +380,7 @@
         eng, P = module._stage_engine()
         S = eng.new_state(P, module.training)
         xs = [t.contiguous().float() for t in tensors[:n_in]]
+        eng.keep_acts = getattr(module, "_keep_state", False)
         outs = module._stage_fwd(eng, P, xs, S)
         if module.training:
             for k, b in module.named_buffers():
```
